# EBonura/bonnie-32

Hardware: AMD Instinct MI355X
Metric: Mtriangles/s + Mpixels/s, 1M-tri synthetic scene @ 2560x1920 (higher is better)
Workload: dtype f32+i32 (exact-order f32 setup/barycentrics, integer snap and RGB555 colour tail); 1 GPU; C3: 1000000 tris @ 2560x1920, 256x256 8-bit atlas, affine+snap+RGB555 dither, painter's; triangles_drawn=485525, fragments=9622635, parallelism=single GPU

## Files before the change

bonnie-32_amd/csrc/b32_api.hip:

```cpp
#include "b32_host.h"
#include "b32_overlay_body.h"

extern "C" {

const char* b32_strerror(int code) {
    switch (code) {
        case B32_OK: return "ok";
        case B32_E_ARG: return "invalid argument";
        case B32_E_INDEX: return "face references a vertex index out of range";
        case B32_E_NAN_KEY: return "NaN painter's-sort key";
        case B32_E_HIP: return "HIP runtime error";
        case B32_E_UNSUPPORTED: return "setting outside the supported hot-path scope";
        case B32_E_NO_DEVICE: return "no HIP device (the rasterizer has no CPU fallback)";
        case B32_E_FRAME_DROPPED: return "an earlier frame in flight ran out of buffer space and drew nothing (deep asynchronous mode)";
        case B32_E_BAND_TIMEOUT: return "a band exchange wait gave up: another rank did not publish / release its frame in time (the frame may hold stale rows)";
        default: return "unknown error";
    }
}

int b32_create(int device, b32_ctx** out) {
    if (!out) return B32_E_ARG;
    *out = nullptr;
    int n = 0;
    if (hipGetDeviceCount(&n) != hipSuccess || n <= 0 || device < 0 || device >= n) return B32_E_NO_DEVICE;
// ... 806 lines not shown
    if ((rc = tmp.alloc(&d_unr, (size_t)K::UNR_ENTRIES))) return rc;
    if ((rc = tmp.alloc(&d_dither, (size_t)16))) return rc;
    launch_constants(c->stream, d_bits, d_unr, d_dither);
    std::vector<uint32_t> h(N);
    HIPCHK(c, hipMemcpyAsync(h.data(), d_bits, N * 4, hipMemcpyDeviceToHost, c->stream));
    if (unr_table257) HIPCHK(c, hipMemcpyAsync(unr_table257, d_unr, K::UNR_ENTRIES, hipMemcpyDeviceToHost, c->stream));
    if (dither16) HIPCHK(c, hipMemcpyAsync(dither16, d_dither, 16 * 4, hipMemcpyDeviceToHost, c->stream));
    HIPCHK(c, hipStreamSynchronize(c->stream));
    for (uint32_t i = 0; i < N && i < cap; ++i) {
        if (names) names[i] = kEntries[i].name;
        if (bits) bits[i] = h[i];
        if (is_f32) is_f32[i] = kEntries[i].f;
    }
    return B32_OK;
}

int b32_last_kernel_times(b32_ctx* c, const char** names, float* ms, uint32_t cap) {
    if (!c || !names || !ms) return 0;
    static const char* const kNames[5] = { "setup", "sort", "bin", "cover", "shade" };
    uint32_t k = 0;
    for (int p = 0; c->phase_frames && p < 5 && k < cap; ++p) {
        if (p != 3 && c->phase_level < 2) continue;
        names[k] = kNames[p]; ms[k] = c->phase_ms[p]; ++k;
    }
    const struct { const char* name; const EventPair* pair; } timers[3] = { { "world_project", &c->world_timer }, { "pick", &c->pick_timer }, { "hover", &c->hover_timer } };
    for (const auto& t : timers) {
        float t_ms = 0.0f;
        if (k < cap && t.pair->elapsed(&t_ms)) { names[k] = t.name; ms[k] = t_ms; ++k; }
    }
    return (int)k;
}

}

extern "C" int b32_set_fragment_counting(b32_ctx* c, int on) {
    if (!c) return B32_E_ARG;
    c->count_fragments = on ? 1 : 0;
    return B32_OK;
}
extern "C" unsigned long long b32_route_count(const b32_ctx* c, int which) {
    if (c && which == 7) return c->pipelined_frames;
    if (c && which == 8) return c->lds_atlas_frames;
    if (c && which == 9) return c->wire_tile_frames;
    if (c && which == 10) return c->span_cover_frames;
    if (c && which == 11) return c->flag_join_frames;
    if (c && which == 12) return c->event_join_frames;
    if (c && which == 13) return c->poll_join_frames;
    if (c && which == 14) return c->lines.tile_batches;
    if (c && which == 15) return c->lines.scan_batches;
    if (c && which == 16) return c->prims.tile_batches;
    if (c && which == 17) return c->prims.scan_batches;
    if (c && which == 18) return c->world_tile_batches;
    if (c && which == 19) return c->world_scan_batches;
    return (c && which >= 0 && which < 8) ? c->routes[which] : 0ull;
}
extern "C" int b32_set_async_depth(b32_ctx* c, int deep) {
    if (!c) return B32_E_ARG;
    if (!deep) { const int rc = settle_pending(c); if (rc) return rc; }
    c->deep_async = deep != 0;
    return B32_OK;
}
extern "C" int b32_set_profiling(b32_ctx* c, int level) {
    if (!c) return B32_E_ARG;
    c->profile_level = level < 0 ? 0 : (level > 2 ? 2 : level);
    if (!c->profile_level) c->hover_timer.timed = c->world_timer.timed = false;
    c->prof_seq = 0;
    if (c->profile_level >= 1 && !c->ev_created) {
        (void)hipSetDevice(c->device);
        for (auto& fr : c->ev) for (auto& e : fr) HIPCHK(c, hipEventCreate(&e));
        c->ev_created = true;
    }
    return B32_OK;
}
extern "C" int b32_set_routes(b32_ctx* c, uint32_t off_mask) {
    if (!c) return B32_E_ARG;
    const int rc = settle_pending(c);
    if (rc) return rc;
    c->route_off = off_mask;
    return B32_OK;
}
extern "C" int b32_set_cheap_threshold(b32_ctx* c, uint32_t den) {
    if (!c || den == 0) return B32_E_ARG;
    c->cheap_den = den;
    c->scene.tex_sig_valid = false;
    return B32_OK;
}
extern "C" int b32_set_pipeline_gate(b32_ctx* c, uint32_t permille) {
    if (!c || permille > 2000u) return B32_E_ARG;
    c->gate_permille = permille;
    return B32_OK;
}
extern "C" int b32_last_shader_clock(const b32_ctx* c, float* ghz, float* fill_ms) {
    if (!c || !ghz) return B32_E_ARG;
    *ghz = 0.0f; if (fill_ms) *fill_ms = 0.0f;
    const unsigned long long* t = c->h_stamps.t;
    if (!t[ST_FILL] || !t[ST_CLKW] || t[ST_CLKW] <= t[ST_FILL] || t[ST_CLK1] <= t[ST_CLK0]) return B32_OK;
    const double ns = (double)(t[ST_CLKW] - t[ST_FILL]) * 10.0;
    *ghz = (float)((double)(t[ST_CLK1] - t[ST_CLK0]) / ns);
    if (fill_ms) *fill_ms = (float)(ns * 1e-6);
    return B32_OK;
}
extern "C" int b32_transparent_counts(const b32_ctx* c, uint32_t* host_bound, uint32_t* device_last) {
    if (!c || !host_bound || !device_last) return B32_E_ARG;
    *host_bound = c->scene.blend_faces; *device_last = c->h_ctrl.n_transparent;
    return B32_OK;
}
// ... 32 lines not shown
```

bonnie-32_amd/csrc/b32_cover.h:

```cpp
#pragma once
#include "b32_fill_common.h"

namespace b32 {

#ifdef B32_TIMELINE
#define B32_DBG_SLOTS(tb) (reinterpret_cast<unsigned long long*>(reinterpret_cast<unsigned char*>(const_cast<uint32_t*>(tb)) + 68096) + (threadIdx.x >> 6) * 32)
#define B32_CLK_DECL(name) unsigned long long name = (unsigned long long)clock64()
#define B32_CLK_ADD(a, slot, from) do { const unsigned long long _n = (unsigned long long)clock64(); if (lane == 0) B32_DBG_SLOTS(tilebuf)[slot] += _n - (from); (from) = _n; } while (0)
#define B32_CNT_ADD(a, slot, v) do { if (lane == 0) B32_DBG_SLOTS(tilebuf)[slot] += (unsigned long long)(v); } while (0)
#else
#define B32_CLK_DECL(name) do { } while (0)
#define B32_CLK_ADD(a, slot, from) do { } while (0)
#define B32_CNT_ADD(a, slot, v) do { } while (0)
#endif

template <int TEXMODE, bool EXACT, bool ZMODE, bool FMT8>
__device__ __forceinline__ uint32_t cover_surface(const Tri& tr, uint32_t cx0, uint32_t cx1, uint32_t cy0, uint32_t cy1, uint32_t li,
                                                  uint32_t* tilebuf, uint32_t x_lo, uint32_t ty_top, uint32_t lane,
                                                  const uint16_t* __restrict__ gtex, const uint16_t* ltex, bool affine) {
    uint32_t drawn_count = 0;
    if (!(tr.flags & F_SLOW)) {
        const uint32_t w = cx1 - cx0, h = cy1 - cy0;
        const uint32_t n88 = ((w + 7) >> 3) * ((h + 7) >> 3), n164 = ((w + 15) >> 4) * ((h + 3) >> 2), n416 = ((w + 3) >> 2) * ((h + 15) >> 4);
        uint32_t sh = 3;
// ... 153 lines not shown
    addr += TRIP; w0 = wa[TRIP - 1] + sa0; w1 = wb[TRIP - 1] + sa1;
}

constexpr float SPAN_MAX_EXT = 512.0f;
constexpr float SPAN_MIN_INV_AREA = 1.0f / 8192.0f;
struct SpanEdge { float r, c; };
__device__ __forceinline__ SpanEdge span_edge(float G) {
    SpanEdge e;
    const float r = __builtin_amdgcn_rcpf(G);
    e.r = G == 0.0f ? -1073741824.0f : r;
    e.c = G == 0.0f ? 64.0f : (G > 0.0f ? -0.5f * r : -0.5f * r + 1.0f);
    return e;
}
__device__ __forceinline__ void span_interval(float E0, float E1, float E2, const SpanEdge& d0, const SpanEdge& d1, const SpanEdge& d2, float wlen,
                                              float& lo, float& hi) {
    const float v0 = __builtin_fmaf(-E0, d0.r, d0.c), v1 = __builtin_fmaf(-E1, d1.r, d1.c), v2 = __builtin_fmaf(-E2, d2.r, d2.c);
    const bool l0 = d0.r > 0.0f, l1 = d1.r > 0.0f, l2 = d2.r > 0.0f;
    lo = fmaxf(fmaxf(l0 ? ceilf(v0) : 0.0f, l1 ? ceilf(v1) : 0.0f), l2 ? ceilf(v2) : 0.0f);
    hi = fminf(fminf(l0 ? wlen : floorf(v0), l1 ? wlen : floorf(v1)), fminf(l2 ? wlen : floorf(v2), wlen));
}
__device__ __forceinline__ void span_trip(unsigned long long* top, unsigned long long* sec, uint32_t addr, uint32_t left, unsigned long long P) {
    constexpr uint32_t TRIP = B32_TRIP;
    if (left) {
        unsigned long long old[TRIP];
#pragma unroll
        for (uint32_t j = 0; j < TRIP; ++j) old[j] = atomicMax(&top[addr + j], j < left ? P : 0ull);
#pragma unroll
        for (uint32_t j = 0; j < TRIP; ++j) atomicMax(&sec[addr + j], j < left ? min(old[j], P) : 0ull);
    }
}

template <int TEXMODE, bool EXACT, int NW, bool ZMODE, bool FMT8, bool P64 = false>
__device__ __forceinline__ unsigned long long phase_a_rows(const FillArgs& a, uint32_t e0, uint32_t n_op, uint32_t lane, uint32_t wave,
                                                           uint32_t* cursor, uint32_t* wmark, const TexDesc& lds_desc,
                                                           uint32_t* tilebuf, const TileRect& rect, const uint16_t* ltex) {
    const uint32_t x_lo = rect.x_lo, x_hi = rect.x_hi, y_lo = rect.y_lo, y_hi = rect.y_hi, ty_top = rect.ty_top;
    const uint16_t* __restrict__ gtex = FMT8 ? reinterpret_cast<const uint16_t*>(a.texels32) : a.texels;
    unsigned long long frags = 0;
    const float ERR = K::ERR;
    const bool affine = a.fp.affine != 0;
    const uint32_t grab_m = max(1u, (n_op + NW * 64u - 1u) / (NW * 64u));
    const uint32_t grab = min(64u, max(4u, (n_op + NW * grab_m - 1u) / (NW * grab_m)));
    for (;;) {
        B32_CLK_DECL(clk);
        uint32_t cs = 0;
        if (lane == 0) cs = atomicAdd(cursor, grab);
        cs = (uint32_t)__builtin_amdgcn_readfirstlane((int)cs);
        if (cs >= n_op) break;
        const uint32_t e = cs + lane;
        bool live = lane < grab && e < n_op;
        Batch b;
        uint32_t my_sid = 0, my_key = 0;
        bool narrow = false;
        load_batch<TEXMODE>(b, a, e0 + e, live, lds_desc, EXACT, ZMODE || (EXACT && !affine), my_sid, my_key, narrow);
        if (ZMODE) { my_key = 0u; my_sid = 0xFFFFFFFEu - my_sid; }
        const uint32_t flags = b.q3.w;
        const uint32_t cx0 = max(b.q1.w & 0xFFFF, x_lo), cx1 = min(b.q1.w >> 16, x_hi);
        const uint32_t cy0 = max(b.q2.x & 0xFFFF, y_lo), cy1 = min(b.q2.x >> 16, y_hi);
        live = live && cx0 < cx1 && cy0 < cy1;
#ifdef B32_TIMELINE
        asm volatile("" :: "v"(cx0), "v"(cy0));
#endif
        B32_CLK_ADD(a, 0, clk); B32_CNT_ADD(a, 4, 1);
        const bool slow = live && (flags & F_SLOW);
        bool span_all = false;
        float sE0 = 0.0f, sE1 = 0.0f;
        uint32_t sG01 = 0, sH01 = 0;
        if (P64 && !EXACT && !ZMODE && a.span_cover) {
            const float fa0 = __uint_as_float(b.q0.z), fb0 = __uint_as_float(b.q0.w), fa1 = __uint_as_float(b.q1.x), fb1 = __uint_as_float(b.q1.y);
            const float inv = __uint_as_float(b.q1.z);
            const float sgn = inv < 0.0f ? -1.0f : 1.0f;
            const float G0 = sgn * fa0, G1 = sgn * fa1, G2 = -(G0 + G1);
            const float H0 = sgn * fb0, H1 = sgn * fb1, H2 = -(H0 + H1);
            const float ext = fmaxf(fmaxf(fmaxf(__builtin_fabsf(G0), __builtin_fabsf(G1)), fmaxf(__builtin_fabsf(H0), __builtin_fabsf(H1))),
                                    fmaxf(__builtin_fabsf(G2), __builtin_fabsf(H2)));
            const float A = __builtin_fabsf(fa0 * fb1 - fb0 * fa1);
            const bool fast = narrow && !(flags & (F_EMPTY | F_SLOW)) && ext <= SPAN_MAX_EXT && __builtin_fabsf(inv) >= SPAN_MIN_INV_AREA && A >= 1.0f;
            span_all = !__ballot(live && !fast);
            const float dx = (float)cx0 - __uint_as_float(b.q0.x), dy = (float)cy0 - __uint_as_float(b.q0.y);
            sE0 = sgn * (fa0 * dx + fb0 * dy); sE1 = sgn * (fa1 * dx + fb1 * dy);
            sG01 = ((uint32_t)hw_cvt_i32(G0) & 0xFFFFu) | ((uint32_t)hw_cvt_i32(G1) << 16);
            sH01 = ((uint32_t)hw_cvt_i32(H0) & 0xFFFFu) | ((uint32_t)hw_cvt_i32(H1) << 16);
        }
        const uint32_t h = (live && !slow) ? cy1 - cy0 : 0u;
        const uint32_t inc = dpp_add_scan(h);
        const uint32_t R = (uint32_t)__builtin_amdgcn_readlane((int)inc, 63);
        const uint32_t P = inc - h;
        const float a0 = __uint_as_float(b.q0.z), b0 = __uint_as_float(b.q0.w), a1 = __uint_as_float(b.q1.x), b1 = __uint_as_float(b.q1.y);
        const uint32_t box = (cx0 - x_lo) | ((cx1 - x_lo) << 8) | ((cy0 - ty_top) << 16);
        const uint32_t boxP = (cx0 - x_lo) | ((cx1 - x_lo) << 6) | ((cy0 - ty_top) << 13) | (P << 19);
        uint32_t lq = 0, lqn = 0;
        auto exact_trip = [&](const Tri& tr, uint32_t& addr, float& w0, float& w1, float sa0, float sa1, float sinv, uint32_t left, unsigned long long P) -> uint32_t {
            unsigned long long* top = reinterpret_cast<unsigned long long*>(tilebuf);
            const uint32_t* mask_l = reinterpret_cast<const uint32_t*>(ltex);
            const bool mask_in_lds = a.mask_lds_words != 0;
            uint32_t drawn = 0;
            float wa[4], wb[4];
            wa[0] = w0; wb[0] = w1;
#pragma unroll
            for (int j = 1; j < 4; ++j) { wa[j] = wa[j - 1] + sa0; wb[j] = wb[j - 1] + sa1; }
            bool in[4]; int ta[4]; unsigned long long Pj[4];
#pragma unroll
            for (int j = 0; j < 4; ++j) {
                const float cx = wa[j] * sinv, cy = wb[j] * sinv;
                const float cz = 1.0f - cx - cy;
                in[j] = ((uint32_t)j < left) & (__builtin_fminf(__builtin_fminf(cx, cy), cz) >= ERR);
                Pj[j] = P; ta[j] = -1;
// ... 330 lines not shown
```

bonnie-32_amd/csrc/b32_device.h:

```cpp
#pragma once
#include <hip/hip_runtime.h>
#include <stdint.h>
#include "../../include/b32raster.h"
#include "b32_world_point.h"

namespace b32 {

constexpr int TILE_W = 64;
constexpr int TILE_H = 64;
constexpr int TILE_STRIDE = 72;
constexpr int FILL_THREADS = 1024;
constexpr int FILL_WAVES = FILL_THREADS / 64;
constexpr uint32_t KEY_INVALID = 0xFFFFFFFFu;

namespace K {
constexpr int      FRAC_BITS = 12;
constexpr float    ONE_F = (float)(1 << FRAC_BITS);
constexpr uint32_t UNR_ENTRIES = 257, UNR_INDEX_OFFSET = 256, UNR_NUMERATOR = 262144, UNR_ROUND_ADD = 1, UNR_ROUND_DIV = 2;
constexpr int32_t  UNR_SUBTRACT = 257;
constexpr uint32_t DIV_D16_SHIFT = 16, DIV_INDEX_SHIFT = 7, DIV_INDEX_MAX = 256, DIV_NR1_SHIFT = 8, DIV_NR2_SHIFT = 8, DIV_SHIFT_BASE = 36;
constexpr uint64_t DIV_INDEX_BIAS = 0x7FC0, DIV_U_ADD = 0x101, DIV_NR1_CONST = 0x2000080, DIV_NR2_CONST = 0x80;
constexpr float    PF_DISTANCE = 5.0f, PF_SCALE = 4.0f, PF_VIEWPORT_DIV = 2.0f, PF_VIEWPORT_FRAC = 0.75f;
constexpr int32_t  PF_DENOM_GUARD = 256;
constexpr float    P_DISTANCE = 5.0f, P_US_SUB = 1.0f, P_VIEWPORT_DIV = 2.0f, P_VIEWPORT_FRAC = 0.75f, P_DENOM_GUARD = 0.001f;
// ... 24 lines not shown
    X("project.distance", F, K::P_DISTANCE) X("project.us_sub", F, K::P_US_SUB) X("project.viewport_div", F, K::P_VIEWPORT_DIV)       \
    X("project.viewport_frac", F, K::P_VIEWPORT_FRAC) X("project.denom_guard", F, K::P_DENOM_GUARD)                                   \
    X("near_plane", F, K::NEAR_PLANE) X("mesh.distance", F, K::MESH_DISTANCE)                                                         \
    X("fill.area_eps", F, K::AREA_EPS) X("fill.err", F, K::ERR) X("fill8.area_eps", F, K::AREA_EPS) X("fill8.err", F, K::ERR)         \
    X("fill.modulate_div", I, K::MOD_DIV) X("fill.modulate_max", I, K::MOD_MAX)                                                       \
    X("fill.shade_clamp_lo", F, K::SHADE_LO) X("fill.shade_clamp_hi", F, K::SHADE_HI) X("fill.shade_max", F, K::SHADE_MAX)            \
    X("fill.nodither_shift", I, K::NODITHER_SHIFT)                                                                                    \
    X("dither.shift", I, K::DITHER_SHIFT) X("dither.clamp_lo", I, K::DITHER_LO) X("dither.clamp_hi", I, K::DITHER_HI)                 \
    X("dither8.shift", I, K::DITHER_SHIFT) X("dither8.clamp_hi", I, K::DITHER_HI) X("dither8.expand_shift", I, K::DITHER8_EXPAND_SHIFT) \
    X("expand5.shl", I, K::EXPAND5_SHL) X("expand5.shr", I, K::EXPAND5_SHR)                                                           \
    X("blend555.in_shift", I, K::BLEND_IN_SHIFT) X("blend555.average_div", I, K::BLEND_AVG_DIV) X("blend555.clamp_hi", I, K::BLEND_HI) \
    X("blend555.clamp_lo", I, K::BLEND_LO) X("blend555.quarter_div", I, K::BLEND_QUARTER_DIV) X("blend555.out_shift", I, K::BLEND_OUT_SHIFT) \
    X("light.min_dist", F, K::LIGHT_MIN_DIST) X("light.color_div", F, K::LIGHT_COLOR_DIV) X("light.total_max", F, K::LIGHT_TOTAL_MAX) \
    X("color15.transparent", I, K::C15_TRANSPARENT) X("color15.black_drawable", I, K::C15_BLACK_DRAWABLE) X("color15.white", I, K::C15_WHITE) \
    X("color15.semi_bit", I, K::C15_SEMI_BIT) X("color15.r_shift", I, K::C15_R_SHIFT) X("color15.g_shift", I, K::C15_G_SHIFT)         \
    X("color15.channel_max", I, K::C15_CHANNEL_MAX)

struct __attribute__((aligned(32))) CovRec {
    uint32_t xy1, xy2, xy3;
    float inv_area;
    uint32_t bbx, bby;
    uint32_t key;
    uint32_t flags;
};
static_assert(sizeof(CovRec) == 32, "CovRec layout");
constexpr uint32_t COV_WIDE = 0x8000u;
struct __attribute__((aligned(64))) ShadeRec {
    float x1, y1, x2, y2;
    float x3, y3, inv_area; uint32_t pk0;
    float u1, u2, u3, v1;
    float v2, v3; uint32_t pk1, pk2;
};
static_assert(sizeof(ShadeRec) == 64, "ShadeRec layout");
constexpr uint32_t SH_BLACK_TR = 1u, SH_DITHER = 2u, SH_SLOW = 4u;
struct __attribute__((aligned(32))) AuxRec {
    float iz1, iz2, iz3, w0_start;
    float w1_start; uint32_t _pad[3];
};
static_assert(sizeof(AuxRec) == 32, "AuxRec layout");

struct RecView { uint4 q0, q1, q2, q3, q4, q5; };
__device__ __forceinline__ float i16lo(uint32_t w) { return (float)(int32_t)(int16_t)(w & 0xFFFFu); }
__device__ __forceinline__ float i16hi(uint32_t w) { return (float)((int32_t)w >> 16); }
__device__ __forceinline__ void view_edges(RecView& r, float x1, float y1, float x2, float y2, float x3, float y3, float inv_area) {
    r.q0 = make_uint4(__float_as_uint(x3), __float_as_uint(y3), __float_as_uint(y2 - y3), __float_as_uint(x3 - x2));
    r.q1.x = __float_as_uint(y3 - y1); r.q1.y = __float_as_uint(x1 - x3); r.q1.z = __float_as_uint(inv_area);
}
__device__ __forceinline__ bool view_from_cov(RecView& r, const uint4& c0, const uint4& c1) {
    r.q1.w = c1.x; r.q2.x = c1.y; r.q3.w = c1.w;
    if ((c0.x & 0xFFFFu) == COV_WIDE) return false;
    view_edges(r, i16lo(c0.x), i16hi(c0.x), i16lo(c0.y), i16hi(c0.y), i16lo(c0.z), i16hi(c0.z), __uint_as_float(c0.w));
    return true;
}
__device__ __forceinline__ void view_edges_from_shade(RecView& r, const uint4& s0, const uint4& s1) {
    view_edges(r, __uint_as_float(s0.x), __uint_as_float(s0.y), __uint_as_float(s0.z), __uint_as_float(s0.w), __uint_as_float(s1.x),
               __uint_as_float(s1.y), __uint_as_float(s1.z));
}
__device__ __forceinline__ uint32_t shade_tex_slot(const uint4& s1, const uint4& s3) { return (s1.w >> 24) | ((s3.z >> 24) << 8); }

constexpr uint32_t F_TEX_MASK   = 0xFFFFu;
constexpr uint32_t F_TEX_NONE   = 0xFFFFu;
constexpr uint32_t F_BLACK_TR   = 1u << 16;
constexpr uint32_t F_BLEND_SHIFT = 17;
constexpr uint32_t F_DITHER     = 1u << 20;
constexpr uint32_t F_SLOW       = 1u << 21;
constexpr uint32_t F_TRANSP     = 1u << 22;
constexpr uint32_t F_EMPTY      = 1u << 23;
constexpr uint32_t F_ALPHA_SHIFT = 24;

struct TexDesc { uint32_t width, height, blend_mode, offset; };

struct Ctrl {
    uint32_t n_visible;
    uint32_t n_transparent;
    uint32_t nan_opaque, nan_transparent;
    uint32_t err_index;
    uint32_t abort;
    uint32_t n_opaque;
    uint32_t n_pairs;
    uint32_t pairs_overflow;
    uint32_t tile_cursor;
    uint32_t list_demand;
    uint32_t need_global_sort;
    uint32_t wire_overflow;
    uint32_t sticky;
    unsigned long long fragments;
};

struct Stamps { unsigned long long t[8]; };
struct Events { uint32_t bad_index, nan_opaque, nan_transparent, overflow, long_transparent, setup_done ,
                join_abort ,
                fill_started ,
                wbin_done ,
                poll_done ,
                poll_lost , _pad[5]; };
__device__ __forceinline__ Events* events_of(Ctrl* ctrl) { return reinterpret_cast<Events*>(reinterpret_cast<unsigned char*>(ctrl) + 128); }
enum { ST_SETUP = 0, ST_BIN = 1, ST_FILL = 2, ST_WIRE = 3, ST_END = 4,
       ST_CLK0 = 5, ST_CLK1 = 6, ST_CLKW = 7 };
__device__ __forceinline__ void phase_stamp(Ctrl* ctrl, int k) {
    if (blockIdx.x == 0 && threadIdx.x == 0) {
        unsigned long long* t = reinterpret_cast<Stamps*>(ctrl + 1)->t;
        if (!t[k]) t[k] = wall_clock64();
    }
}

constexpr uint32_t LOCAL_SORT_CAP = 2048;
// ... 110 lines not shown
    __device__ __forceinline__ bool inside(uint32_t px, uint32_t py) const { return (px < x_hi) & ((py >= y_lo) & (py < y_hi)); }
};
__device__ __forceinline__ TileRect tile_rect(const FrameParams& fp, uint32_t tile) {
    TileRect r;
    r.x_lo = (tile % fp.tiles_x) * TILE_W; r.x_hi = min(r.x_lo + TILE_W, fp.width);
    tile_row_geom(fp, tile / fp.tiles_x, r.ty_top, r.th);
    r.y_lo = max(r.ty_top, fp.band_y0); r.y_hi = min(r.ty_top + r.th, fp.band_y1);
    return r;
}
__device__ __forceinline__ uint32_t pack_tile_span(uint32_t bbx, uint32_t bby, uint32_t flags, const FrameParams& fp, uint32_t& count) {
    count = 0;
    if (flags & F_EMPTY) return 0xFFFFFFFFu;
    const uint32_t min_x = bbx & 0xFFFF, max_x = bbx >> 16;
    const uint32_t min_y = max(bby & 0xFFFF, fp.band_y0), max_y = min(bby >> 16, fp.band_y1);
    if (min_x >= max_x || min_y >= max_y) return 0xFFFFFFFFu;
    const uint32_t tx0 = min_x / TILE_W, tx1 = (max_x - 1) / TILE_W;
    const uint32_t ty0 = tile_row_of(fp, min_y), ty1 = tile_row_of(fp, max_y - 1);
    count = (tx1 - tx0 + 1) * (ty1 - ty0 + 1);
    return tx0 | (tx1 << 8) | (ty0 << 16) | (ty1 << 24);
}

struct SortScratch {
    uint32_t* block_hist;
    uint32_t  max_blocks;
    uint32_t* digit_total;
};
constexpr int SORT_THREADS = 256;
constexpr int SORT_ITEMS = 16;
constexpr int SORT_TILE = SORT_THREADS * SORT_ITEMS;

struct RadixExtra {
    Ctrl* post_ctrl = nullptr; const uint32_t* partials = nullptr; uint32_t npart = 0;
    uint32_t* ranges_out = nullptr; uint32_t n_ranges = 0;
};
void launch_radix_pass(hipStream_t s, const uint32_t* keys_in, const uint32_t* vals_in, uint32_t* keys_out, uint32_t* vals_out,
                       const uint32_t* n_dev, uint32_t n_cap, int shift, int bits, const SortScratch& sc, const RadixExtra& ex = RadixExtra());

constexpr uint32_t LIGHTS_INLINE = 8;
struct LightSet { B32Light l[LIGHTS_INLINE]; };
constexpr uint32_t BATCH_MESHES = 32;
struct MeshRow { float ambient; uint32_t flags; B32Fog fog; };
struct MeshTable { MeshRow m[BATCH_MESHES]; };
constexpr uint32_t ROW_CULL = 1u, ROW_FOG = 2u, ROW_PLACED = 4u;
struct PlaceTable { B32Placement p[BATCH_MESHES]; };
static_assert(sizeof(B32Placement) == 20 && sizeof(PlaceTable) == 640, "B32Placement layout");
struct RecArrays { CovRec* cov; ShadeRec* shade; AuxRec* aux; };
#ifndef B32_FILL_PAD
#define B32_FILL_PAD 32
#endif
constexpr uint32_t FILL_PAD = B32_FILL_PAD;
struct DirectBin {
    uint32_t* fill;
    uint32_t* lists;
    uint32_t region, cap_opaque, cap_transparent;
    uint32_t with_class;
    uint32_t epoch;
};
void launch_merge_mesh(hipStream_t s, const B32Vertex* sv, uint32_t nv, const B32Face* sf, uint32_t nf, uint32_t nt, B32Vertex* dv, B32Face* df,
                       uint32_t vbase, uint32_t tbase, uint32_t mesh);
void launch_offset_tex(hipStream_t s, const TexDesc* src, uint32_t nt, TexDesc* dst, uint32_t texel_base);
struct SetupBuffers {
    const B32Vertex* verts;
    const B32Face* faces;
    const TexDesc* tex;
    const B32Light* lights;
    RecArrays recs;
    DirectBin db;
    float* shades;
    uint32_t* keys;
    uint32_t* spans;
    uint32_t* partials;
    Ctrl* ctrl;
    WireTri* wire;
    const float* pos12;
    const float* attr12;
    uint32_t* face_of;
};
struct SetupArgs {
    FrameParams fp;
    SetupBuffers buf;
    LightSet lset;
    MeshTable mtab;
    PlaceTable ptab;
};
void launch_setup(hipStream_t s, const SetupArgs& a);
void launch_gate(hipStream_t s, Ctrl* prev, uint32_t need, uint32_t patience_ticks, uint32_t start_seq, Ctrl* mine, uint32_t start_patience_ticks = 200000000u);
void launch_flag(hipStream_t s, Ctrl* ctrl, uint32_t epoch);
void launch_flag_poll(hipStream_t s, Ctrl* ctrl, uint32_t seq);
void launch_flag_wbin(hipStream_t s, Ctrl* ctrl, uint32_t epoch);
void launch_join(hipStream_t s, Ctrl* ctrl, uint32_t epoch, uint32_t patience_ticks);
void launch_pack_streams(hipStream_t s, const B32Vertex* verts, uint32_t nv, float* pos12, float* attr12, bool with_lit);
void launch_pose_rest(hipStream_t s, const B32Vertex* verts, uint32_t nv, float* rest);
void launch_pose(hipStream_t s, const float* rest, const uint16_t* bone_of, B32Vertex* verts, uint32_t nv, const B32Bone* bones, uint32_t n_bones);
void launch_project_fixed(hipStream_t s, const float* pos, uint32_t n, B32Camera cam, uint32_t w, uint32_t h,
                          int32_t* sx, int32_t* sy, float* z);
void launch_selftest(hipStream_t s, int op, const float* a, const float* b, const float* c, float* out, uint32_t n);
void launch_constants(hipStream_t s, uint32_t* consts, uint8_t* unr, int32_t* dither);
void launch_build_mask(hipStream_t s, const uint16_t* texels15, const uint32_t* texels32, uint32_t n, uint32_t* mask);
constexpr uint32_t MASK_LDS_MAX_WORDS = 9216;
void launch_clear(hipStream_t s, uint32_t* fb, size_t n_px, uint32_t rgba);
struct UploadSegs { void* dst[16]; uint32_t src_off[16]; uint32_t n16[16]; uint32_t count; };
void launch_upload(hipStream_t s, const void* arena_dev, const UploadSegs& segs);
void launch_ctrl_out(hipStream_t s, Ctrl* ctrl, void* dst128);
void launch_expand_indexed(hipStream_t s, const uint8_t* idx, uint32_t n, const uint16_t* clut, uint32_t clut_len, uint16_t* out, uint32_t* skippable);

void launch_bin(hipStream_t s, const FrameParams& fp, const uint32_t* spans, const uint32_t* order, Ctrl* ctrl,
// ... 63 lines not shown
    const float* pos; uint32_t stride, nv;
    const HoverHalfEdge* he; const uint32_t* poly_start; const uint32_t* poly_verts; uint32_t np, nh;
    OverlayPoint* tab;
    OverlayBounds* bounds;
    const uint32_t* selected; uint32_t n_sel;
    B32MeshOverlay o;
    uint32_t at_brackets, at_edges, at_dots, at_hover_vertex, at_hover_edge, at_hover_face, at_selected, at_preview;
    uint32_t hover_face_cnt;
    uint32_t g_edges, g_pedges, g_sel, g_pfaces, g_hover, g_brackets;
};
void launch_overlay(hipStream_t s, const OverlayArgs& a);
constexpr uint32_t BLEND_SORT_CAP = 2048;
bool bin_spans_applicable(const FrameParams& fp, const SortScratch& sc, bool with_class);
bool launch_bin_spans(hipStream_t s, const FrameParams& fp, const uint32_t* spans, const uint32_t* keys, const uint32_t* partials, Ctrl* ctrl,
                      const SortScratch& sc, uint32_t pair_cap, uint32_t* ranges, uint32_t* tile_mid, uint32_t blend_cap, uint32_t* pair_vals);
void launch_tile_ranges(hipStream_t s, const uint32_t* pair_keys, const Ctrl* ctrl, uint32_t pair_cap, uint32_t* ranges, uint32_t n_keys);

void launch_clear_gradient(hipStream_t s, uint32_t* fb, float* zbuf, uint32_t width, uint32_t height, uint32_t y0, uint32_t y1, uint32_t top, uint32_t bottom);
void launch_sky(hipStream_t s, const B32SkyVertex* v, uint32_t nv, const uint32_t* faces, uint32_t nf, const B32Camera& cam, float2* proj,
                uint32_t* fb, uint32_t width, uint32_t height, uint32_t band_y0, uint32_t band_y1);
void launch_stars(hipStream_t s, const int32_t* cx, const int32_t* cy, const uint8_t* rgb, uint32_t n, float size, uint32_t* fb,
                  uint32_t width, uint32_t height, uint32_t band_y0, uint32_t band_y1);
void launch_upscale_nearest(hipStream_t s, const uint32_t* src, uint32_t sw, uint32_t sh, uint32_t* dst, uint32_t dw, uint32_t dh);

struct FillArgs {
    FrameParams fp;
    const CovRec* crecs;
    const ShadeRec* srecs;
    const AuxRec* xrecs;
    const float* shades;
    uint32_t* pair_vals;
    const uint32_t* keys;
    uint32_t local_sort;
    const uint32_t* ranges;
    uint32_t* tile_mid;
    uint32_t tile_keys_only;
    const TexDesc* tex;
    const uint16_t* texels;
    uint32_t* fb;
    float* zbuf;
    uint32_t* vis;
    TexDesc tex0;
    Ctrl* ctrl;
    uint32_t lds_tex_texels;
    uint32_t may_blend;
    uint32_t exact_coverage;
    uint32_t skip_solid;
    const uint32_t* texels32;
    uint32_t ordered_all;
    uint32_t gather_blend;
    uint32_t inline_bin;
    uint32_t direct_bin;
    uint32_t* tile_fill;
    uint32_t epoch;
    uint32_t list_stride;
    const uint32_t* spans;
    const uint32_t* partials;
    const uint32_t* texmask;
    uint32_t mask_lds_words;
    uint32_t clear_on, clear_rgba;
    uint32_t clear_depth;
    uint32_t wide;
    const uint8_t* atlas0;
    uint32_t atlas_idx_bytes;
    uint32_t stagger;
    uint32_t span_cover;
    uint32_t join_seq, join_patience;
    uint32_t start_seq;
    uint32_t start_defer;
    uint32_t fused;
#ifdef B32_TIMELINE
    unsigned long long* dbg;
#endif
};
void launch_fill(hipStream_t s, const FillArgs& a, int n_cu, hipEvent_t after_cover = nullptr);
size_t fill_lds_tex_budget();
constexpr uint32_t ATLAS_CLUT_BYTES = 512;
uint32_t fill_lds_atlas_room(bool wide);

}
```

bonnie-32_amd/csrc/b32_fill.hip:

```cpp
#include "b32_cover.h"
#include "b32_shade_tile.h"

namespace b32 {

constexpr uint32_t RQ_WORDS = 64, RQ_BYTES = RQ_WORDS * 4;
static_assert(2 * (4 * LDS_TILE_BYTES + LDS_MISC_BYTES + 8 * RQ_BYTES + 511) / 512 * 512 <= 160 * 1024, "two 8-wave workgroups per CU");

template <int NT>
__device__ __forceinline__ void reduce_setup_counters(const FillArgs& a, uint32_t* misc, uint32_t tid, uint32_t lane) {
    if (tid < 5) misc[8 + tid] = 0;
    __syncthreads();
    const uint32_t npart = (a.fp.nf + 255) / 256;
    uint32_t acc[5] = { 0, 0, 0, 0, 0 };
    for (uint32_t b = tid; b < npart; b += NT)
#pragma unroll
        for (int k = 0; k < 5; ++k) acc[k] += a.partials[b * 8 + k];
#pragma unroll
    for (int k = 0; k < 5; ++k) {
        const uint32_t tot = (uint32_t)__builtin_amdgcn_readlane((int)dpp_add_scan(acc[k]), 63);
        if (lane == 0 && tot) atomicAdd(&misc[8 + k], tot);
    }
    __syncthreads();
    if (tid == 0) {
        const uint32_t t[5] = { misc[8], misc[9], misc[10], misc[11], misc[12] };
// ... 37 lines not shown
        const unsigned long long t0 = wall_clock64();
        uint32_t lost = 0, waited = 0;
        while (__hip_atomic_fetch_add(&ev->poll_done, 0u, __ATOMIC_RELAXED, __HIP_MEMORY_SCOPE_AGENT) != a.join_seq) {
            if (wall_clock64() - t0 > (unsigned long long)a.join_patience) { lost = 1; break; }
            waited = 1;
            __builtin_amdgcn_s_sleep(32);
        }
        if (lost) { atomicOr(&a.ctrl->sticky, 8u); (void)__hip_atomic_exchange(&ev->poll_lost, a.join_seq, __ATOMIC_RELAXED, __HIP_MEMORY_SCOPE_AGENT); }
        if (waited) __builtin_amdgcn_fence(__ATOMIC_ACQUIRE, "agent");
        misc[7] = lost;
    }
    __syncthreads();
    return misc[7] != 0;
}

template <int NT>
__device__ __forceinline__ TexDesc stage_texture(const FillArgs& a, unsigned char* dst_bytes, uint32_t tid) {
    const TexDesc lds_desc = a.tex[0];
    const uint4* src = reinterpret_cast<const uint4*>(a.texels + lds_desc.offset);
    uint4* dst = reinterpret_cast<uint4*>(dst_bytes);
    const uint32_t nq = (a.lds_tex_texels + 7) / 8;
    for (uint32_t i = tid; i < nq; i += NT) dst[i] = src[i];
    return lds_desc;
}

template <int NT>
__device__ __forceinline__ void leave_undrawn(const FillArgs& a, uint32_t ntiles, uint32_t tid, uint32_t redraw, bool publish) {
    if (a.direct_bin) {
        for (uint32_t t = blockIdx.x * NT + tid; t < ntiles; t += gridDim.x * NT) {
            uint32_t* fl = a.tile_fill + (size_t)t * FILL_PAD;
            if (redraw & 2u) atomicMax(&a.ctrl->list_demand, fl[0]);
            fl[0] = 0; fl[1] = 0;
        }
        if (blockIdx.x == 0 && tid == 0 && publish) a.ctrl->need_global_sort = redraw;
    }
    if (a.clear_on) clear_band<NT>(a);
}

__device__ __forceinline__ void staggered_start(const FillArgs& a) {
    if (blockIdx.x >= gridDim.x / 2) {
        const unsigned long long t0 = wall_clock64();
        while (wall_clock64() - t0 < (unsigned long long)a.stagger) __builtin_amdgcn_s_sleep(8);
    }
}

template <int TEXMODE, int NT, bool P64>
__device__ __forceinline__ bool tile_list_range(const FillArgs& a, uint32_t tile, uint32_t* tilebuf, uint32_t* sort_cnt, uint32_t* misc, uint32_t tid,
                                                uint32_t& e0, uint32_t& e1) {
    if (P64 && a.inline_bin) {
        e0 = e1 = tile * a.list_stride;
    } else if (P64 && a.direct_bin) {
        const uint32_t* fl = a.tile_fill + (size_t)tile * FILL_PAD;
        const uint32_t n_o = fl[0], n_t = fl[1];
        e0 = tile * a.list_stride; e1 = e0 + n_o;
        if (tid == 0) {
            if (a.gather_blend) a.tile_mid[tile] = e0 + a.list_stride - n_t;
            if (n_o | n_t) atomicAdd(&a.ctrl->n_pairs, n_o + n_t);
        }
    } else if (P64) {
        e0 = a.ranges[tile]; e1 = a.gather_blend ? a.tile_mid[tile] : a.ranges[tile + 1];
    } else if (TEXMODE == 0 && a.local_sort) {
        e0 = a.ranges[tile];
        const uint32_t e2 = a.ranges[tile + 1];
        if (e2 - e0 > LOCAL_SORT_CAP) {
            if (tid == 0) atomicOr(&a.ctrl->need_global_sort, 1u);
            __syncthreads();
            return false;
        }
        if (e2 > e0) [[clang::noinline]] tile_local_sort<NT>(tilebuf, sort_cnt, misc + 8, a.keys, a.pair_vals + e0, e2 - e0, &misc[4]);
        e1 = e0 + misc[4];
        if (tid == 0) a.tile_mid[tile] = e1;
    } else {
        e0 = a.ranges[2 * tile]; e1 = a.ranges[2 * tile + 1];
    }
    return true;
}

template <int NT>
__device__ __forceinline__ void collect_tile_list(const FillArgs& a, uint32_t tile, uint32_t e0, uint32_t* misc, uint32_t pre_span, uint32_t pre_key,
                                                  uint32_t tid, uint32_t lane) {
    const FrameParams& fp = a.fp;
    const uint32_t txi = tile % fp.tiles_x, tyl = tile / fp.tiles_x;
    const uint32_t r_end = e0 + a.list_stride;
    for (uint32_t f0 = 0; f0 < fp.nf; f0 += NT) {
        const uint32_t f = f0 + tid;
        bool hit = false, tr = false;
        if (f < fp.nf) {
            const uint32_t span = f0 == 0 ? pre_span : a.spans[f];
            hit = span != 0xFFFFFFFFu && txi >= (span & 0xFF) && txi <= ((span >> 8) & 0xFF) && tyl >= ((span >> 16) & 0xFF) && tyl <= (span >> 24);
            if (hit && a.gather_blend) tr = ((f0 == 0 ? pre_key : a.keys[f]) >> 31) != 0;
        }
        const unsigned long long mo = __ballot(hit && !tr), mt = __ballot(hit && tr);
        uint32_t bo = 0, bt = 0;
        if (lane == 0 && mo) bo = atomicAdd((&misc[4]), (uint32_t)__builtin_popcountll(mo));
        if (lane == 0 && mt) bt = atomicAdd((&misc[5]), (uint32_t)__builtin_popcountll(mt));
        bo = (uint32_t)__builtin_amdgcn_readfirstlane((int)bo); bt = (uint32_t)__builtin_amdgcn_readfirstlane((int)bt);
        const unsigned long long below = (1ull << lane) - 1ull;
        if (hit && !tr) a.pair_vals[e0 + bo + (uint32_t)__builtin_popcountll(mo & below)] = f;
        if (hit && tr) a.pair_vals[r_end - 1u - (bt + (uint32_t)__builtin_popcountll(mt & below))] = f;
    }
}

template <bool EXACT, int NT, bool ZMODE, bool P64>
__device__ __forceinline__ void seed_planes(const FillArgs& a, uint32_t* tilebuf, const TileRect& rect, uint32_t tid) {
    const FrameParams& fp = a.fp;
    if (P64 && ZMODE) {
        unsigned long long* t64 = reinterpret_cast<unsigned long long*>(tilebuf);
        for (uint32_t p = tid; p < TILE_W * rect.th; p += NT) {
            const uint32_t row = p >> 6, col = p & 63;
// ... 362 lines not shown
```

bonnie-32_amd/csrc/b32_fill_common.h:

```cpp
#pragma once
#include "b32_device.h"
#ifndef B32_TRIP
#define B32_TRIP 4
#endif
#ifndef B32_DRAIN_TRIPS
#define B32_DRAIN_TRIPS 2
#endif
static_assert(B32_DRAIN_TRIPS > 0, "row remainders are queued and worked off at most B32_DRAIN_TRIPS trips per round");
#ifndef B32_P64_WAVES
#define B32_P64_WAVES 4
#endif
#ifndef B32_P64_STRIDE
#define B32_P64_STRIDE 66
#endif

namespace b32 {

constexpr int LDS_TILE_BYTES = TILE_H * TILE_STRIDE * 4;
constexpr int STR64 = B32_P64_STRIDE;
static_assert(STR64 >= 64 && STR64 <= TILE_STRIDE && (TILE_H - 1) * STR64 + 64 + 4 <= TILE_H * TILE_STRIDE, "64-bit planes must fit their allocation, trip overshoot included");
constexpr int LDS_MISC_BYTES = 64;
constexpr int LDS_MARK_BYTES = FILL_WAVES * 64 * 4;
constexpr int LDS_TEX_OFFSET = 2 * LDS_TILE_BYTES + LDS_MISC_BYTES + LDS_MARK_BYTES;
constexpr int LDS_SORT_CNT_BYTES = 8 * 256 * 4;
// ... 187 lines not shown
            case B32_BLEND_ADD_QUARTER: r = min(b + f / 4, 255); break;
            case B32_BLEND_ERASE:       r = 0; a8 = 0; break;
        }
        ps1 |= (uint32_t)r << (8 * i);
    }
    if (alpha < 255) {
        const float a = (float)alpha / 255.0f, inv_a = 1.0f - a;
        uint32_t o = 0xFF000000u;
#pragma unroll
        for (int i = 0; i < 3; ++i)
            o |= f2u8_sat((float)((ps1 >> (8 * i)) & 255) * a + (float)((back >> (8 * i)) & 255) * inv_a) << (8 * i);
        return o;
    }
    return ps1 | (a8 << 24);
}

__device__ __forceinline__ void replay_w(const Tri& t, uint32_t px, uint32_t py, float& w0, float& w1) {
    float r0 = t.w0_start, r1 = t.w1_start;
    for (uint32_t y = t.min_y; y < py; ++y) { r0 += t.b0; r1 += t.b1; }
    for (uint32_t x = t.min_x; x < px; ++x) { r0 += t.a0; r1 += t.a1; }
    w0 = r0; w1 = r1;
}
__device__ __forceinline__ void edge_w(const Tri& t, uint32_t px, uint32_t py, float& w0, float& w1) {
    if (!(t.flags & F_SLOW)) {
        const float dx = (float)px - t.x3, dy = (float)py - t.y3;
        w0 = t.a0 * dx + t.b0 * dy; w1 = t.a1 * dx + t.b1 * dy;
    } else replay_w(t, px, py, w0, w1);
}

struct Batch {
    uint4 q0, q1, q2, q3, q4, q5;
    uint32_t tw, th, toff;
};

__device__ __forceinline__ void load_shade_view(const FillArgs& a, uint32_t sid, bool need5, RecView& r) {
    const uint4* sp = reinterpret_cast<const uint4*>(a.srecs + sid);
    const uint4 s0 = sp[0], s1 = sp[1], s2 = sp[2], s3 = sp[3];
    view_edges_from_shade(r, s0, s1);
    r.q1.w = 0; r.q2.x = 0;
    r.q2.y = s2.x; r.q2.z = s2.y; r.q2.w = s2.z;
    r.q3.x = s2.w; r.q3.y = s3.x; r.q3.z = s3.y;
    const uint32_t sh = s3.w >> 24;
    r.q3.w = shade_tex_slot(s1, s3) | ((sh & SH_BLACK_TR) ? F_BLACK_TR : 0u) | ((sh & SH_DITHER) ? F_DITHER : 0u) | ((sh & SH_SLOW) ? F_SLOW : 0u) |
             (255u << F_ALPHA_SHIFT);
    r.q4 = make_uint4(s1.w & 0xFFFFFFu, s3.z & 0xFFFFFFu, s3.w & 0xFFFFFFu, 0u);
    r.q5 = make_uint4(0, 0, 0, 0);
    if (need5 || (sh & SH_SLOW)) {
        const uint4* xp = reinterpret_cast<const uint4*>(a.xrecs + sid);
        const uint4 x0 = xp[0], x1 = xp[1];
        r.q4.w = x0.w; r.q5 = make_uint4(x1.x, x0.x, x0.y, x0.z);
    }
    if (sh & SH_SLOW) { const uint4 c1 = reinterpret_cast<const uint4*>(a.crecs + sid)[1]; r.q1.w = c1.x; r.q2.x = c1.y; }
}
__device__ __forceinline__ void load_full_view(const FillArgs& a, uint32_t sid, RecView& r) {
    load_shade_view(a, sid, true, r);
    const uint4 c1 = reinterpret_cast<const uint4*>(a.crecs + sid)[1];
    r.q1.w = c1.x; r.q2.x = c1.y; r.q3.w = c1.w;
}

template <int TEXMODE>
__device__ __forceinline__ void load_batch(Batch& b, const FillArgs& a, uint32_t entry, bool live, const TexDesc& lds_desc, bool need_uv,
                                           bool need_aux, uint32_t& sid_out, uint32_t& key_out, bool& narrow_out) {
    b.q0 = b.q1 = b.q2 = b.q3 = b.q4 = b.q5 = make_uint4(0, 0, 0, 0);
    b.tw = b.th = b.toff = 0;
    sid_out = 0; key_out = 0; narrow_out = false;
    if (live) {
        const uint32_t sid = a.pair_vals[entry];
        const uint4* cp = reinterpret_cast<const uint4*>(a.crecs + sid);
        const uint4 c0 = cp[0], c1 = cp[1];
        sid_out = sid; key_out = c1.z;
        RecView v;
        v.q0 = v.q1 = v.q2 = v.q3 = v.q4 = v.q5 = make_uint4(0, 0, 0, 0);
        const bool narrow = view_from_cov(v, c0, c1);
        narrow_out = narrow;
        if (!narrow || need_uv) {
            const uint4* sp = reinterpret_cast<const uint4*>(a.srecs + sid);
            const uint4 s0 = sp[0], s1 = sp[1];
            if (!narrow) view_edges_from_shade(v, s0, s1);
            if (need_uv) {
                const uint4 s2 = sp[2], s3 = sp[3];
                v.q2.y = s2.x; v.q2.z = s2.y; v.q2.w = s2.z;
                v.q3.x = s2.w; v.q3.y = s3.x; v.q3.z = s3.y;
                v.q4 = make_uint4(s1.w & 0xFFFFFFu, s3.z & 0xFFFFFFu, s3.w & 0xFFFFFFu, 0u);
                const uint32_t tid = c1.w & F_TEX_MASK;
                if (tid != F_TEX_NONE) {
                    if (TEXMODE == 1) { b.tw = lds_desc.width; b.th = lds_desc.height; b.toff = 0; }
                    else { const TexDesc d = a.tex[tid]; b.tw = d.width; b.th = d.height; b.toff = d.offset; }
                }
            }
        }
        if (need_aux || (c1.w & F_SLOW)) {
            const uint4* xp = reinterpret_cast<const uint4*>(a.xrecs + sid);
            const uint4 x0 = xp[0], x1 = xp[1];
            v.q4.w = x0.w; v.q5 = make_uint4(x1.x, x0.x, x0.y, x0.z);
        }
        b.q0 = v.q0; b.q1 = v.q1; b.q2 = v.q2; b.q3 = v.q3; b.q4 = v.q4; b.q5 = v.q5;
    }
}
__device__ __forceinline__ Tri tri_from_batch(const Batch& b, int t, bool full) {
    Tri r;
    r.x3 = bcf(__uint_as_float(b.q0.x), t); r.y3 = bcf(__uint_as_float(b.q0.y), t);
    r.a0 = bcf(__uint_as_float(b.q0.z), t); r.b0 = bcf(__uint_as_float(b.q0.w), t);
    r.a1 = bcf(__uint_as_float(b.q1.x), t); r.b1 = bcf(__uint_as_float(b.q1.y), t);
    r.inv_area = bcf(__uint_as_float(b.q1.z), t);
    const uint32_t bbx = bcu(b.q1.w, t), bby = bcu(b.q2.x, t);
    r.min_x = bbx & 0xFFFF; r.max_x = bbx >> 16; r.min_y = bby & 0xFFFF; r.max_y = bby >> 16;
    r.flags = bcu(b.q3.w, t);
    r.u1 = r.u2 = r.u3 = r.v1 = r.v2 = r.v3 = 0.0f; r.tw = r.th = r.toff = 0; r.w0_start = r.w1_start = 0.0f;
    if (full) {
        r.u1 = bcf(__uint_as_float(b.q2.y), t); r.u2 = bcf(__uint_as_float(b.q2.z), t); r.u3 = bcf(__uint_as_float(b.q2.w), t);
        r.v1 = bcf(__uint_as_float(b.q3.x), t); r.v2 = bcf(__uint_as_float(b.q3.y), t); r.v3 = bcf(__uint_as_float(b.q3.z), t);
        r.tw = bcu(b.tw, t); r.th = bcu(b.th, t); r.toff = bcu(b.toff, t);
    }
    if (r.flags & F_SLOW) { r.w0_start = bcf(__uint_as_float(b.q4.w), t); r.w1_start = bcf(__uint_as_float(b.q5.x), t); }
    r.iz1 = r.iz2 = r.iz3 = 0.0f;
    if (full) { r.iz1 = bcf(__uint_as_float(b.q5.y), t); r.iz2 = bcf(__uint_as_float(b.q5.z), t); r.iz3 = bcf(__uint_as_float(b.q5.w), t); }
    return r;
}
__device__ __forceinline__ Tri tri_from_view(const RecView& r, bool with_uv) {
    Tri t;
    t.x3 = __uint_as_float(r.q0.x); t.y3 = __uint_as_float(r.q0.y); t.a0 = __uint_as_float(r.q0.z); t.b0 = __uint_as_float(r.q0.w);
    t.a1 = __uint_as_float(r.q1.x); t.b1 = __uint_as_float(r.q1.y); t.inv_area = __uint_as_float(r.q1.z);
    t.min_x = r.q1.w & 0xFFFF; t.max_x = r.q1.w >> 16; t.min_y = r.q2.x & 0xFFFF; t.max_y = r.q2.x >> 16;
    t.flags = r.q3.w;
    t.w0_start = __uint_as_float(r.q4.w); t.w1_start = __uint_as_float(r.q5.x);
    t.u1 = t.u2 = t.u3 = t.v1 = t.v2 = t.v3 = 0.0f; t.iz1 = t.iz2 = t.iz3 = 0.0f; t.tw = t.th = t.toff = 0;
    if (with_uv) {
        t.u1 = __uint_as_float(r.q2.y); t.u2 = __uint_as_float(r.q2.z); t.u3 = __uint_as_float(r.q2.w);
        t.v1 = __uint_as_float(r.q3.x); t.v2 = __uint_as_float(r.q3.y); t.v3 = __uint_as_float(r.q3.z);
        t.iz1 = __uint_as_float(r.q5.y); t.iz2 = __uint_as_float(r.q5.z); t.iz3 = __uint_as_float(r.q5.w);
    }
    return t;
}
template <bool EXACT, bool ZMODE>
__device__ __forceinline__ void commit_fragment(uint32_t* tilebuf, uint32_t addr, uint32_t li, uint32_t zkey) {
    if (ZMODE) atomicMin(reinterpret_cast<unsigned long long*>(tilebuf) + addr, ((unsigned long long)zkey << 32) | li);
    else if (EXACT) atomicMax(&tilebuf[addr], li);
    else {
        const uint32_t old = atomicMax(&tilebuf[addr], li);
        atomicMax(&tilebuf[addr + TILE_H * TILE_STRIDE], min(old, li));
    }
}
__device__ __forceinline__ bool frag_zkey(const Tri& t, float bcx, float bcy, float bcz, uint32_t& zkey) {
    const float inv_z = bcx * t.iz1 + bcy * t.iz2 + bcz * t.iz3;
    const float z = rcp_exact(inv_z);
    zkey = zsort_key(z);
    return z == z;
}

__device__ inline float exact_depth_at(const FillArgs& a, uint32_t sid, uint32_t px, uint32_t py) {
    RecView rv;
    load_full_view(a, sid, rv);
    const Tri tr = tri_from_view(rv, true);
    float w0, w1, bcx, bcy, bcz;
    edge_w(tr, px, py, w0, w1);
    (void)inside_bc(tr, w0, w1, bcx, bcy, bcz);
    const float inv_z = bcx * tr.iz1 + bcy * tr.iz2 + bcz * tr.iz3;
    return rcp_exact(inv_z);
}

struct Hit { float bcx, bcy, bcz; uint32_t texel, vc1, vc2, vc3, flags, sid; };
template <bool FMT8>
__device__ __forceinline__ bool hit_test(const FillArgs& a, uint32_t sid, uint32_t px, uint32_t py, Hit& h) {
    RecView rv;
    load_shade_view(a, sid, a.fp.affine == 0, rv);
    Tri tr = tri_from_view(rv, true);
    const uint32_t txid = tr.flags & F_TEX_MASK;
    if (txid != F_TEX_NONE) {
        if (a.fp.nt == 1) { tr.tw = a.tex0.width; tr.th = a.tex0.height; tr.toff = a.tex0.offset; }
        else { const TexDesc d = a.tex[txid]; tr.tw = d.width; tr.th = d.height; tr.toff = d.offset; }
    }
    float w0, w1;
    edge_w(tr, px, py, w0, w1);
    if (!inside_bc(tr, w0, w1, h.bcx, h.bcy, h.bcz)) return false;
    h.texel = 0;
    if (!texel_drawn<0, FMT8>(tr, h.bcx, h.bcy, h.bcz, FMT8 ? reinterpret_cast<const uint16_t*>(a.texels32) : a.texels, nullptr, h.texel, a.fp.affine != 0)) return false;
    h.vc1 = rv.q4.x; h.vc2 = rv.q4.y; h.vc3 = rv.q4.z; h.flags = tr.flags; h.sid = sid;
    return true;
}
template <bool FMT8>
__device__ __forceinline__ uint32_t colour(const FillArgs& a, const Hit& h, int shading, uint32_t px, uint32_t py) {
    float shv[9];
    if (shading != B32_SHADE_NONE) for (int j = 0; j < 9; ++j) shv[j] = a.shades[(size_t)h.sid * 9 + j];
    if (FMT8) return (shade8(h.texel, h.bcx, h.bcy, h.bcz, h.vc1, h.vc2, h.vc3, h.flags, shading, shv, px, py) & 0xFFFFFFu) | 0xFF000000u;
    return shade15<true>(h.texel, h.bcx, h.bcy, h.bcz, h.vc1, h.vc2, h.vc3, h.flags, shading, shv, px, py);
}

using RecRegs = RecView;
__device__ __forceinline__ void rec_load(const FillArgs& a, uint32_t sid, bool need5, RecRegs& r) { load_shade_view(a, sid, need5, r); }
__device__ __forceinline__ bool hit_prepare(const FillArgs& a, const RecRegs& r, uint32_t px, uint32_t py, Hit& h, int& taddr) {
    Tri tr = tri_from_view(r, true);
    float w0, w1;
    edge_w(tr, px, py, w0, w1);
    taddr = -1;
    if (!inside_bc(tr, w0, w1, h.bcx, h.bcy, h.bcz)) return false;
    h.vc1 = r.q4.x; h.vc2 = r.q4.y; h.vc3 = r.q4.z; h.flags = tr.flags;
    const uint32_t txid = tr.flags & F_TEX_MASK;
    if (txid == F_TEX_NONE) return true;
    TexDesc d;
    if (a.fp.nt == 1) d = a.tex0; else d = a.tex[txid];
    if (d.width == 0 || d.height == 0) { taddr = -2; return true; }
    float u, v;
    interp_uv(h.bcx, h.bcy, h.bcz, tr.u1, tr.u2, tr.u3, tr.v1, tr.v2, tr.v3, tr.iz1, tr.iz2, tr.iz3, a.fp.affine != 0, u, v);
    taddr = (int)(d.offset + texel_index(u, v, d.width, d.height));
    return true;
// ... 63 lines not shown
```

bonnie-32_amd/csrc/b32_frame.hip:

```cpp
#include "b32_host.h"

static void swap_with(b32_ctx* c, FrameSet& a) { std::swap(c->cur, a); }
static void rotate_sets(b32_ctx* c) {
    swap_with(c, c->alt[0]);
    if (c->n_sets == 3) std::swap(c->alt[0], c->alt[1]);
}
static void unrotate_sets(b32_ctx* c) {
    if (c->n_sets == 3) std::swap(c->alt[0], c->alt[1]);
    swap_with(c, c->alt[0]);
}
static int pipeline_ensure(b32_ctx* c) {
    if (!c->side) {
        int prio_least = 0, prio_greatest = 0;
        (void)hipDeviceGetStreamPriorityRange(&prio_least, &prio_greatest);
        HIPCHK(c, hipStreamCreateWithPriority(&c->side, hipStreamNonBlocking, prio_least));
        HIPCHK(c, hipEventCreateWithFlags(&c->ev_main, hipEventDisableTiming));
        HIPCHK(c, hipEventCreateWithFlags(&c->ev_wbin, hipEventDisableTiming));
        HIPCHK(c, hipEventCreateWithFlags(&c->cur.ev_setup, hipEventDisableTiming));
        for (FrameSet& a : c->alt) HIPCHK(c, hipEventCreateWithFlags(&a.ev_setup, hipEventDisableTiming));
        c->side_dirty = true;
    }
    for (uint32_t k = 0; k + 1 < c->n_sets; ++k) {
        FrameSet& a = c->alt[k];
        if (!a.d_ctrl) {
            HIPCHK(c, hipMalloc(reinterpret_cast<void**>(&a.d_ctrl), sizeof(Ctrl) + sizeof(Stamps) + sizeof(Events)));
            HIPCHK(c, hipMemsetAsync(a.d_ctrl, 0, sizeof(Ctrl) + sizeof(Stamps) + sizeof(Events), c->stream));
            c->side_dirty = true;
        }
        if (a.cap_work < c->cap_work || !a.crecs) {
            HIPCHK(c, hipStreamSynchronize(c->stream));
            a.release();
            const size_t n = c->cap_work;
            int rc;
            if ((rc = ensure_plain(c, a.keys0, n))) return rc;
            if ((rc = ensure_plain(c, a.crecs, n))) return rc;
            if ((rc = ensure_plain(c, a.srecs, n))) return rc;
            if ((rc = ensure_plain(c, a.xrecs, n))) return rc;
            if ((rc = ensure_plain(c, a.spans, n))) return rc;
            if ((rc = ensure_plain(c, a.face_of, n))) return rc;
            if ((rc = ensure_plain(c, a.partials, (size_t)((n + 255) / 256) * 8 + 8))) return rc;
            a.cap_work = n;
        }
    }
    return B32_OK;
}

extern "C" {
int validate_settings(const B32Settings* st) {
    if (st->shading > B32_SHADE_GOURAUD) return B32_E_ARG;
    if (st->n_lights && !st->lights) return B32_E_ARG;
    if (st->shading != B32_SHADE_NONE)
        for (uint32_t i = 0; i < st->n_lights; ++i)
            if (st->lights[i].enabled && st->lights[i].type > B32_LIGHT_SPOT) return B32_E_ARG;
    return B32_OK;
}

static uint32_t bits_for(uint32_t n_keys) { uint32_t b = 1; while ((1ull << b) < n_keys) ++b; return b; }

struct FramePlan {
    bool wire_back = false, wire_front = false;
    bool with_class = false;
    bool ordered_all = false;
    bool want_prio64 = false;
    bool exact_cov = false;
    bool local_sort = false;
    bool want_inline = false;
    bool direct_bin = false;
    bool inline_bin = false, prio64 = false;
    uint32_t list_stride = 0;
    DirectBin db{};
    uint32_t ntiles = 0;
    bool fused = false, wide = false;
    void set_prio64(bool on) { prio64 = on; fused = plan_fused(prio64, wire_front, ordered_all); }
    HandOver hand_over_kind = HandOver::None;
    hipStream_t setup_stream = nullptr;
    uint32_t poll_seq = 0, poll_patience = 0;
    uint32_t start_seq = 0;
    bool wire_on = false, wire_binned = false, wire_polled = false;
    WireArgs wa{};
    const float *pos12 = nullptr, *attr12 = nullptr;
    bool prof_all = false, prof_fill = false;
    hipEvent_t* ev = nullptr;
    int pair_buf = 0;
};

struct SetsGuard {
    b32_ctx* c; bool armed = false;
    explicit SetsGuard(b32_ctx* ctx) : c(ctx) {}
    SetsGuard(const SetsGuard&) = delete;
    SetsGuard& operator=(const SetsGuard&) = delete;
    void rotate() { rotate_sets(c); armed = true; }
    void dismiss() { armed = false; }
    ~SetsGuard() { if (armed) { unrotate_sets(c); c->pipelined = false; } }
};

static FrameParams frame_params(const b32_ctx* c, const B32Camera* cam, const B32Settings* st, const B32Fog* fog, bool wire_any) {
    FrameParams fp{};
    fp.cam = *cam;
    fp.width = c->width; fp.height = c->height;
    fp.band_y0 = c->band_y0; fp.band_y1 = c->band_y1;
    fp.tiles_x = (c->width + TILE_W - 1) / TILE_W;
    fp.tile_h = TILE_H;
    fp.tile_yb = (c->band_y0 / TILE_H) * TILE_H;
    fp.tiles_y = c->band_y1 > c->band_y0 ? (c->band_y1 - fp.tile_yb + TILE_H - 1) / TILE_H : 0;
    fp.nv = c->scene.nv; fp.nf = c->scene.nf; fp.nt = c->scene.nt;
    fp.n_lights = st->shading != B32_SHADE_NONE ? st->n_lights : 0;
    fp.ambient = st->ambient;
    fp.affine = st->affine_textures; fp.shading = st->shading; fp.backface_cull = st->backface_cull;
    fp.dithering = st->dithering; fp.fixed_point = st->use_fixed_point; fp.has_fog = fog ? 1 : 0; fp.zmode = st->use_zbuffer ? 1 : 0;
    if (fog) fp.fog = *fog;
    fp.camfx = make_camfx_any(*cam, c->width, c->height);
    fp.fmt8 = c->scene.fmt8 ? 1 : 0;
    fp.ortho = st->has_ortho ? 1 : 0; fp.xray = st->xray_mode ? 1 : 0;
    fp.ortho_zoom = st->ortho_zoom; fp.ortho_cx = st->ortho_center_x; fp.ortho_cy = st->ortho_center_y;
    fp.wire_collect = wire_any ? 1 : 0;
    fp.band_only = 0;
    fp.redraw = c->redrawing ? 1 : 0;
    fp.tex_blend_any = c->scene.tex_blend_any ? 1 : 0;
    fp.batched = c->frame_batched ? 1 : 0;
    fp.placed = c->frame_placed ? 1 : 0;
// ... 74 lines not shown
            if (wt > c->cur.cap_wire_tiles || !c->cur.wire_fill) {
                if ((rc = ensure_plain(c, c->cur.wire_fill, (wt + 2) * FILL_PAD + 64))) return rc;
                if ((rc = ensure_plain(c, c->cur.wire_lists, wt * WIRE_TILE_CAP + 64))) return rc;
                c->cur.cap_wire_tiles = wt; c->cur.wire_grid = 0;
            }
            const unsigned long long grid = ((unsigned long long)c->width << 40) ^ ((unsigned long long)c->band_y0 << 20) ^ c->band_y1;
            if (grid != c->cur.wire_grid) {
                HIPCHK(c, hipMemsetAsync(c->cur.wire_fill, 0, ((c->cur.cap_wire_tiles + 2) * FILL_PAD + 64) * sizeof(uint32_t), s));
                c->cur.wire_grid = grid; c->side_dirty = true;
            }
        }
    }
    return B32_OK;
}

static int plan_route(b32_ctx* c, FrameParams& fp, const SortScratch& sc, FramePlan& r) {
    const bool wire_front = r.wire_front;
    int rc;
    r.with_class = c->scene.may_blend && !c->scene.fmt8;
    const bool spans_ok = !(c->route_off & B32_ROUTE_SORT_FREE) && c->scene.local_sort_ok && bin_spans_applicable(fp, sc, r.with_class);
    r.ordered_all = c->scene.fmt8 ? c->scene.blend8 : (fp.xray != 0);
    r.want_prio64 = spans_ok && !fp.ortho && !r.ordered_all;
    if (r.want_prio64 && !(c->route_off & B32_ROUTE_CUT_TILES)) {
        static_assert(PLAN_TILE_H == (uint32_t)TILE_H, "b32_frame_plan.h cuts the tiles of b32_device.h");
        const TileGrid g = plan_cut_grid(fp.tiles_x, c->band_y0, c->band_y1, (uint32_t)c->n_cu, (uint32_t)B32_MIN_TILE_H);
        fp.tile_h = g.tile_h; fp.tile_yb = g.tile_yb; fp.tiles_y = g.tiles_y;
    }
    const uint32_t ntiles = r.ntiles = fp.tiles_x * fp.tiles_y;
    r.exact_cov = c->count_fragments || !c->scene.cheap_ok || (fp.zmode && !r.want_prio64);
    r.local_sort = !r.exact_cov && c->scene.local_sort_ok && !fp.ortho && !r.ordered_all && !fp.zmode;
    fp.band_only = (r.want_prio64 && c->band_set) ? 1 : 0;
    r.list_stride = (c->scene.nf + 31u) & ~31u;
    r.want_inline = r.want_prio64 && !wire_front && c->scene.nf <= (r.with_class ? 2048u : 8192u) && (size_t)ntiles * r.list_stride <= ((size_t)4 << 20) &&
                    !(c->route_off & B32_ROUTE_INLINE_BIN);
    if (c->scene.direct_ntiles != ntiles) { c->scene.direct_ntiles = ntiles; c->scene.direct_cap_opaque = 0; c->scene.direct_ok = true; }
    if (r.want_prio64 && !r.want_inline && !wire_front && c->scene.direct_ok && !(c->route_off & B32_ROUTE_DIRECT_BIN) && ntiles) {
        if (!c->scene.direct_cap_opaque) c->scene.direct_cap_opaque = std::max<uint32_t>(512u, (uint32_t)std::min<uint64_t>((uint64_t)3 * c->scene.nf / ntiles + 64, 1u << 24));
        if (c->scene.nf <= 65536u && (uint64_t)ntiles * (c->scene.nf + (r.with_class ? BLEND_SORT_CAP : 0u)) <= (8u << 20)) c->scene.direct_cap_opaque = std::max(c->scene.direct_cap_opaque, c->scene.nf);
        const uint32_t cap_o = (c->scene.direct_cap_opaque + 31u) & ~31u;
        const uint32_t region = cap_o + (r.with_class ? BLEND_SORT_CAP : 0u);
        const size_t need = (size_t)ntiles * region + 64;
        if (need <= ((size_t)1 << 28)) {
            if (need > c->cur.cap_direct || !c->cur.direct_lists) {
                if ((rc = ensure_plain(c, c->cur.direct_lists, need + need / 8))) return rc;
                c->cur.cap_direct = need + need / 8;
            }
            const size_t need_fill = (size_t)ntiles * FILL_PAD + 64;
            if (need_fill > c->cur.cap_tile_fill || !c->cur.tile_fill) {
                if ((rc = ensure_plain(c, c->cur.tile_fill, need_fill * 2))) return rc;
                c->cur.cap_tile_fill = need_fill * 2;
                HIPCHK(c, hipMemsetAsync(c->cur.tile_fill, 0, c->cur.cap_tile_fill * sizeof(uint32_t), c->stream));
                c->side_dirty = true;
            }
            if (++c->epoch == 0) c->epoch = 1;
            r.db.fill = c->cur.tile_fill; r.db.lists = c->cur.direct_lists; r.db.region = region; r.db.cap_opaque = cap_o;
            r.db.cap_transparent = r.with_class ? BLEND_SORT_CAP : 0u; r.db.with_class = r.with_class ? 1u : 0u; r.db.epoch = c->epoch;
            r.direct_bin = true;
            r.list_stride = region;
        } else c->scene.direct_ok = false;
    }
    if (!r.direct_bin && r.want_inline) {
        const size_t need = (size_t)ntiles * r.list_stride + 64;
        if (need > c->cap_inline) {
            if ((rc = ensure_plain(c, c->inline_lists, need + need / 2))) return rc;
            c->cap_inline = need + need / 2;
        }
        r.inline_bin = true;
    }
    r.set_prio64(r.direct_bin || r.inline_bin);
    return B32_OK;
}

static int frame_positions(b32_ctx* c, const FrameParams& fp, const float*& pos12, const float*& attr12) {
    int rc;
    pos12 = attr12 = nullptr;
    if (c->scene.nv && c->scene.nf > 8192u && !(c->route_off & B32_ROUTE_PACKED_STREAMS)) {
        const bool want_lit = fp.shading != B32_SHADE_NONE;
        if ((!c->scene.pos_valid || (want_lit && !c->scene.lit_valid)) && c->scene.band_frames >= 1) {
            const bool with_lit = want_lit || c->scene.lit_valid;
            const size_t need = (size_t)c->scene.nv * (with_lit ? 12 : 6);
            if (need > c->scene.cap_pos12 || !c->scene.d_pos12) {
                if ((rc = ensure_plain(c, c->scene.d_pos12, need + 16))) return rc;
                c->scene.cap_pos12 = need;
            }
            launch_pack_streams(c->stream, c->scene.d_verts, c->scene.nv, c->scene.d_pos12, c->scene.d_pos12 + (size_t)c->scene.nv * 3, with_lit);
            c->scene.pos_valid = true; c->scene.lit_valid = with_lit; c->side_dirty = true;
        }
        c->scene.band_frames++;
        if (c->scene.pos_valid && (!want_lit || c->scene.lit_valid)) { pos12 = c->scene.d_pos12; attr12 = c->scene.d_pos12 + (size_t)c->scene.nv * 3; }
    }
    return B32_OK;
}

static int bin_keyed(b32_ctx* c, const FrameParams& fp, FramePlan& r, const SortScratch& sc, hipEvent_t ev_bin) {
    hipStream_t s = c->stream;
    const uint32_t ntiles = r.ntiles;
    int& cur = r.pair_buf;
    cur = 0;
    if (r.local_sort) {
        if (ev_bin) HIPCHK(c, hipEventRecord(ev_bin, s));
        launch_bin_faces(s, fp, c->cur.spans, c->cur.keys0, c->cur.partials, c->cur.d_ctrl, c->pkeys[0], c->pvals[0], (uint32_t)c->cap_pairs, 0);
    } else {
        RadixExtra ex1; ex1.post_ctrl = c->cur.d_ctrl; ex1.partials = c->cur.partials; ex1.npart = (c->scene.nf + 255) / 256;
        launch_radix_pass(s, c->cur.keys0, nullptr, c->keys1, c->vals[1], c->scene.d_consts, c->scene.nf, 0, 8, sc, ex1);
        launch_radix_pass(s, c->keys1, c->vals[1], c->cur.keys0, c->vals[0], &c->cur.d_ctrl->n_visible, c->scene.nf, 8, 8, sc);
        launch_radix_pass(s, c->cur.keys0, c->vals[0], c->keys1, c->vals[1], &c->cur.d_ctrl->n_visible, c->scene.nf, 16, 8, sc);
        launch_radix_pass(s, c->keys1, c->vals[1], c->cur.keys0, c->vals[0], &c->cur.d_ctrl->n_visible, c->scene.nf, 24, 8, sc);
        if (fp.ortho) {
            launch_class_keys(s, c->cur.crecs, c->vals[0], &c->cur.d_ctrl->n_visible, c->scene.nf, c->cur.keys0);
            launch_radix_pass(s, c->cur.keys0, c->vals[0], c->keys1, c->vals[1], &c->cur.d_ctrl->n_visible, c->scene.nf, 0, 8, sc);
            HIPCHK(c, hipMemcpyAsync(c->vals[0], c->vals[1], (size_t)c->scene.nf * 4, hipMemcpyDeviceToDevice, s));
        }
        if (ev_bin) HIPCHK(c, hipEventRecord(ev_bin, s));
        launch_bin(s, fp, c->cur.spans, c->vals[0], c->cur.d_ctrl, c->counts, c->block_sums, c->bin_blocks, c->pkeys[0], c->pvals[0], (uint32_t)c->cap_pairs);
    }
    const uint32_t n_sort_keys = r.local_sort ? ntiles : 2 * ntiles;
    const uint32_t kb = bits_for(n_sort_keys ? n_sort_keys : 1);
    if (kb <= 8 || kb > 12) {
        for (uint32_t shift = 0; shift < kb; shift += 8) {
            launch_radix_pass(s, c->pkeys[cur], c->pvals[cur], c->pkeys[cur ^ 1], c->pvals[cur ^ 1], &c->cur.d_ctrl->n_pairs, (uint32_t)c->cap_pairs, (int)shift, 8, sc);
            cur ^= 1;
        }
        launch_tile_ranges(s, c->pkeys[cur], c->cur.d_ctrl, (uint32_t)c->cap_pairs, c->ranges, n_sort_keys);
    } else {
        RadixExtra exr; exr.ranges_out = c->ranges; exr.n_ranges = n_sort_keys + 1;
        launch_radix_pass(s, c->pkeys[cur], c->pvals[cur], c->pkeys[cur ^ 1], c->pvals[cur ^ 1], &c->cur.d_ctrl->n_pairs, (uint32_t)c->cap_pairs, 0, kb <= 11 ? 11 : 12, sc, exr);
        cur ^= 1;
    }
    return B32_OK;
}

static FillArgs fill_args(const b32_ctx* c, const FrameParams& fp, const FramePlan& r) {
    FillArgs fa{};
    fa.fp = fp; fa.crecs = c->cur.crecs; fa.srecs = c->cur.srecs; fa.xrecs = c->cur.xrecs; fa.shades = c->cur.shades; fa.pair_vals = c->pvals[r.pair_buf]; fa.ranges = c->ranges;
    fa.keys = c->cur.keys0; fa.local_sort = r.local_sort ? 1u : 0u; fa.tile_keys_only = (r.local_sort || r.prio64) ? 1u : 0u; fa.tile_mid = c->tile_mid;
    fa.tex = c->scene.d_tex; fa.texels = c->scene.d_texels; fa.fb = c->fb; fa.vis = c->vis; fa.zbuf = c->zbuf; fa.ctrl = c->cur.d_ctrl;
    fa.tex0 = c->scene.nt ? c->scene.h_tex[0] : TexDesc{ 0, 0, 0, 0 };
    fa.lds_tex_texels = 0;
    if (c->scene.nt == 1 && r.exact_cov) {
        const size_t n = (size_t)c->scene.h_tex[0].width * c->scene.h_tex[0].height;
        if (n > 0 && n * 2 <= fill_lds_tex_budget()) fa.lds_tex_texels = (uint32_t)n;
    }
    fa.exact_coverage = r.exact_cov ? 1u : 0u;
    fa.may_blend = c->scene.may_blend ? 1u : 0u;
    fa.skip_solid = r.wire_front ? 1u : 0u;
    fa.texels32 = c->scene.d_texels32;
    fa.ordered_all = r.ordered_all ? 1u : 0u;
    fa.fused = r.fused ? 1u : 0u;
    fa.wide = r.wide ? 1u : 0u;
    fa.texmask = c->scene.d_texmask;
    { const uint32_t words = c->scene.pool_texels / 32 + 2; fa.mask_lds_words = (c->scene.pool_texels && words <= MASK_LDS_MAX_WORDS) ? words : 0u; }
    fa.inline_bin = r.inline_bin ? 1u : 0u; fa.list_stride = r.list_stride; fa.spans = c->cur.spans; fa.partials = c->cur.partials;
    if (r.inline_bin) fa.pair_vals = c->inline_lists;
    fa.direct_bin = r.direct_bin ? 1u : 0u; fa.tile_fill = c->cur.tile_fill; fa.epoch = c->epoch;
    if (r.direct_bin) fa.pair_vals = c->cur.direct_lists;
    fa.gather_blend = (r.prio64 && r.with_class) ? 1u : 0u;
    fa.stagger = (c->route_off & B32_ROUTE_STAGGER) ? 0u : 1u;
    fa.span_cover = (r.prio64 && !r.exact_cov && !fp.zmode && !(c->route_off & B32_ROUTE_SPAN_COVER)) ? 1u : 0u;
    fa.atlas0 = c->scene.d_atlas0; fa.atlas_idx_bytes = 0;
    if (r.prio64 && !c->scene.fmt8 && c->scene.nt == 1 && c->scene.atlas_idx_bytes && !(c->route_off & B32_ROUTE_LDS_ATLAS) &&
        c->scene.atlas_idx_bytes + ATLAS_CLUT_BYTES + 16u <= fill_lds_atlas_room(r.wide))
        fa.atlas_idx_bytes = c->scene.atlas_idx_bytes;
    if (c->scene.fmt8) fa.fp.xray = 0;
    return fa;
}

static int choose_frame_set(b32_ctx* c, const FramePlan& r, SetsGuard& sets) {
    c->pipelined = false;
    const uint32_t pipe_min_faces = 2048u;
    if (!(c->frame_pending && c->pipe_hint && !c->redrawing && !r.prof_all && c->scene.nf > pipe_min_faces && !(c->route_off & B32_ROUTE_PIPELINE) &&
          c->stream != hipStreamLegacy))
        return B32_OK;
    int rc;
    if ((rc = pipeline_ensure(c))) return rc;
    sets.rotate();
    c->pipelined = true;
    if (c->join_stream != c->stream) {
        int pm = 0, ps = 0;
        c->join_ok = hipStreamGetPriority(c->stream, &pm) == hipSuccess && hipStreamGetPriority(c->side, &ps) == hipSuccess && pm != ps;
        c->join_stream = c->stream;
    }
    return B32_OK;
}

static int profiling_row(b32_ctx* c, FramePlan& r) {
    if (!r.prof_fill) return B32_OK;
    if (!c->ev_created) {
        for (auto& fr : c->ev) for (auto& e : fr) if (hipEventCreate(&e) != hipSuccess) return B32_E_HIP;
        c->ev_created = true;
    }
    r.ev = c->ev[c->ev_frames % EV_RING];
    return B32_OK;
}

static void plan_pipeline(b32_ctx* c, const FrameParams& fp, FramePlan& r) {
    const bool join_small = !c->frame_batched && (c->join_stream != c->stream || c->join_ok);
    c->pipe_hint = plan_pipe_hint(r.direct_bin, r.ntiles, (uint32_t)c->n_cu, c->frame_batched, join_small);
    if (!c->pipe_hint) c->pipelined = false;
    c->last_local_sort = r.local_sort || r.want_prio64;
    c->last_exact = r.ordered_all ? true : (r.exact_cov && !fp.zmode);
    c->last_direct = r.direct_bin;
    const bool narrow_only = (c->route_off & B32_ROUTE_WIDE_GROUPS) != 0;
    r.wide = plan_wide(r.ntiles, (uint32_t)c->n_cu, narrow_only);
    r.hand_over_kind = plan_hand_over({ c->pipelined, c->frame_batched, c->join_ok, r.direct_bin, r.wire_front, r.ordered_all, r.ntiles, (uint32_t)c->n_cu, narrow_only });
}

static int reset_ctrl_of_empty_frame(b32_ctx* c) {
    if (c->scene.nf) return B32_OK;
// ... 47 lines not shown
    b.recs = RecArrays{ c->cur.crecs, c->cur.srecs, c->cur.xrecs }; b.db = r.db;
    b.shades = c->cur.shades; b.keys = c->cur.keys0;
    b.spans = r.direct_bin ? nullptr : c->cur.spans;
    b.partials = c->cur.partials; b.ctrl = c->cur.d_ctrl; b.wire = c->cur.wire;
    b.pos12 = r.pos12; b.attr12 = r.attr12; b.face_of = c->cur.face_of;
    return a;
}

static bool take_lost_flag(b32_ctx* c) {
    const bool lose_flag = (c->inject & 1u) != 0;
    c->inject &= ~1u;
    return lose_flag;
}

static int hand_over(b32_ctx* c, FramePlan& r) {
    hipStream_t s = c->stream;
    if (r.hand_over_kind == HandOver::Poll) {
        const bool lose_flag = take_lost_flag(c);
        if (++c->join_seq == 0) c->join_seq = 1;
        launch_flag_poll(c->side, c->cur.d_ctrl, lose_flag ? c->join_seq ^ 0x40000000u : c->join_seq);
        r.poll_seq = c->join_seq; r.poll_patience = lose_flag ? PATIENCE_INJECTED_TICKS : PATIENCE_TICKS;
        c->flag_join_frames++; c->poll_join_frames++;
    } else if (r.hand_over_kind == HandOver::FlagJoin) {
        const bool lose_flag = take_lost_flag(c);
        launch_flag(c->side, c->cur.d_ctrl, lose_flag ? c->epoch ^ 0x40000000u : c->epoch);
        launch_join(s, c->cur.d_ctrl, c->epoch, lose_flag ? PATIENCE_INJECTED_TICKS : PATIENCE_TICKS);
        c->flag_join_frames++;
    } else if (r.hand_over_kind == HandOver::Event) {
        hipError_t e1 = hipEventRecord(c->cur.ev_setup, c->side);
        if (e1 == hipSuccess) e1 = hipStreamWaitEvent(s, c->cur.ev_setup, 0);
        if (e1 != hipSuccess) { (void)hipStreamSynchronize(c->side); c->last_hip = (int)e1; return B32_E_HIP; }
        c->event_join_frames++;
    }
    if (c->pipelined && r.wire_on && r.wa.tile_fill) {
        launch_wire_bin(c->side, r.wa, r.wire_back, r.wire_front, true);
        if (r.wire_back) { launch_flag_wbin(c->side, c->cur.d_ctrl, r.wa.epoch); r.wire_polled = true; }
        else HIPCHK(c, hipEventRecord(c->ev_wbin, c->side));
        r.wire_binned = true;
    }
    c->cur.in_flight = true;
    if (r.prof_all) HIPCHK(c, hipEventRecord(r.ev[1], s));
    return B32_OK;
}

static int tile_lists(b32_ctx* c, const FrameParams& fp, const SortScratch& sc, FramePlan& r) {
    hipStream_t s = c->stream;
    int rc;
    if (r.prof_all && r.want_prio64) HIPCHK(c, hipEventRecord(r.ev[2], s));
    if (r.want_prio64 && !r.prio64)
        r.set_prio64(launch_bin_spans(s, fp, c->cur.spans, r.with_class ? c->cur.keys0 : nullptr, c->cur.partials, c->cur.d_ctrl, sc, (uint32_t)c->cap_pairs, c->ranges,
                                      c->tile_mid, BLEND_SORT_CAP, c->pvals[0]));
    if (!r.prio64 && (rc = bin_keyed(c, fp, r, sc, r.prof_all ? r.ev[2] : nullptr))) return rc;
    c->routes[r.direct_bin ? 0 : r.inline_bin ? 1 : r.prio64 ? 2 : 3]++;
    const bool direct_safe = r.direct_bin && r.db.cap_opaque >= c->scene.nf && (!r.with_class || c->scene.blend_faces <= BLEND_SORT_CAP);
    c->pending_may_redraw = !(r.inline_bin || direct_safe);
    if (r.prof_fill) HIPCHK(c, hipEventRecord(r.ev[3], s));
    return B32_OK;
}

static int fill(b32_ctx* c, const FrameParams& fp, FramePlan& r) {
    const bool fused = r.fused;
    int rc;
    FillArgs fa = fill_args(c, fp, r);
    if (++c->fill_seq == 0) c->fill_seq = 1;
    fa.start_seq = r.start_seq = c->fill_seq;
    fa.join_seq = r.poll_seq; fa.join_patience = r.poll_patience;
    if ((c->inject & 2u) && fused && r.ntiles) { c->inject &= ~2u; fa.start_seq = 0; c->start_lost = true; }
    fa.start_defer = (fused && r.ntiles > 2u * (uint32_t)c->n_cu && fa.gather_blend) ? 1u : 0u;
    if (c->clear_pending) {
        const bool has_z = c->zbuf && c->zbuf_valid;
        if (fused && (!has_z || fp.zmode) && c->scene.nf && r.ntiles && c->clear_y0 == c->band_y0 && c->clear_y1 == c->band_y1) {
            fa.clear_on = 1; fa.clear_rgba = c->clear_rgba; fa.clear_depth = (has_z && fp.zmode) ? 1u : 0u; c->clear_pending = false;
        } else if ((rc = flush_clear(c))) return rc;
    }
    if (fa.atlas_idx_bytes && fused) c->lds_atlas_frames++;
    if (fa.span_cover && fused) c->span_cover_frames++;
    launch_fill(c->stream, fa, c->n_cu, r.prof_fill ? r.ev[4] : nullptr);
    return B32_OK;
}

static int wire_phases(b32_ctx* c, FramePlan& r) {
    hipStream_t s = c->stream;
    if (r.wire_on && r.wire_binned && !r.wire_polled) HIPCHK(c, hipStreamWaitEvent(s, c->ev_wbin, 0));
    if (r.wire_on) launch_wire(s, r.wa, r.wire_back, r.wire_front, r.wire_binned, r.wire_polled ? c->cur.d_ctrl : nullptr, r.wa.epoch);
    if (r.prof_all) HIPCHK(c, hipEventRecord(r.ev[5], s));
    if (r.prof_fill) c->ev_frames++;
    return B32_OK;
}

static void remember_cover(b32_ctx* c, const FramePlan& r) {
    const uint32_t tiles = r.fused ? r.ntiles : 0u;
    b32_ctx::CoverOf* slot = &c->cover_of[0];
    for (auto& co : c->cover_of) { if (co.ctrl == c->cur.d_ctrl) { slot = &co; break; } if (!co.ctrl) slot = &co; }
    *slot = { c->cur.d_ctrl, tiles, std::min<uint32_t>(r.ntiles, (uint32_t)c->n_cu * 2u), tiles ? r.start_seq : 0u };
}

int enqueue_frame(b32_ctx* c, const B32Camera* cam, const B32Settings* st, const B32Fog* fog) {
    FramePlan r;
    r.wire_back = st->backface_cull && st->backface_wireframe;
    r.wire_front = st->wireframe_overlay != 0;
    FrameParams fp = frame_params(c, cam, st, fog, r.wire_back || r.wire_front);
    LightSet lset{};
    r.prof_fill = c->profile_level >= 1 && (c->prof_seq++ % c->prof_stride) == 0;
    r.prof_all = r.prof_fill && c->profile_level >= 2;
    int rc;
    SetsGuard sets(c);
// ... 197 lines not shown
```

bonnie-32_amd/csrc/b32_frame_plan.h:

```cpp
#pragma once
#include <cstdint>

namespace b32 {

constexpr uint32_t PATIENCE_TICKS = 200000000u;
constexpr uint32_t PATIENCE_INJECTED_TICKS = 200000u;

constexpr uint32_t PLAN_TILE_H = 64;
struct TileGrid { uint32_t tile_h, tile_yb, tiles_y; };
inline TileGrid plan_cut_grid(uint32_t tiles_x, uint32_t band_y0, uint32_t band_y1, uint32_t n_cu, uint32_t min_tile_h) {
    uint32_t th = PLAN_TILE_H;
    if (band_y1 <= band_y0) return { th, (band_y0 / th) * th, 0u };
    while (th > min_tile_h && tiles_x * ((band_y1 + th - 1) / th - band_y0 / th) < (th == PLAN_TILE_H ? 2u : 1u) * n_cu &&
           (band_y1 - band_y0) / (th / 2) + 2 <= 255 ) th /= 2;
    const uint32_t yb = (band_y0 / th) * th;
    return { th, yb, (band_y1 - yb + th - 1) / th };
}

inline uint32_t plan_gate_need(uint32_t gate_permille, uint32_t tiles, uint32_t groups) {
    if (!gate_permille || !tiles) return 0u;
    const uint32_t pre = tiles > groups ? tiles - groups : 0u;
    return gate_permille > 1000u ? (uint32_t)((uint64_t)(gate_permille - 1000u) * pre / 1000u)
                                 : pre + (uint32_t)((uint64_t)(gate_permille - 1u) * groups / 1000u);
}

inline bool plan_fused(bool prio64, bool wire_front, bool ordered_all) { return prio64 && !wire_front && !ordered_all; }

inline bool plan_wide(uint32_t ntiles, uint32_t n_cu, bool narrow_only) { return ntiles <= n_cu && !narrow_only; }

inline bool plan_pipe_hint(bool direct_bin, uint32_t ntiles, uint32_t n_cu, bool batched, bool join_small) {
    return direct_bin && (ntiles > 2u * n_cu || batched || join_small);
}

enum class HandOver {
    None,
    Poll,
    FlagJoin,
    Event
};
struct HandOverIn {
    bool pipelined;
    bool batched;
    bool join_ok;
    bool direct_bin, wire_front, ordered_all;
    uint32_t ntiles, n_cu;
    bool narrow_only;
};
inline HandOver plan_hand_over(const HandOverIn& in) {
    if (!in.pipelined) return HandOver::None;
    if (in.batched && in.join_ok && plan_fused(in.direct_bin, in.wire_front, in.ordered_all) && in.ntiles && 8u * in.ntiles <= 5u * in.n_cu &&
        !in.narrow_only)
        return HandOver::Poll;
    if (in.direct_bin && in.join_ok && !in.batched) return HandOver::FlagJoin;
    return HandOver::Event;
}

}
```

bonnie-32_amd/csrc/b32_host.h:

```cpp
#pragma once
#include "b32_device.h"
#include "b32_frame_plan.h"
#include <algorithm>
#include <cstdio>
#include <chrono>
#include <cstring>
#include <vector>

using namespace b32;
#ifndef B32_MIN_TILE_H
#define B32_MIN_TILE_H 8
#endif

namespace {
constexpr int EV_RING = 64;
constexpr int EV_PER_FRAME = 6;
}

struct FrameSet {
    uint32_t* keys0 = nullptr; CovRec* crecs = nullptr; ShadeRec* srecs = nullptr; AuxRec* xrecs = nullptr;
    uint32_t* spans = nullptr; uint32_t* partials = nullptr; size_t cap_work = 0;
    uint32_t* face_of = nullptr;
    float* shades = nullptr; size_t cap_shades = 0;
    uint32_t* direct_lists = nullptr; size_t cap_direct = 0;
    uint32_t* tile_fill = nullptr; size_t cap_tile_fill = 0;
    WireTri* wire = nullptr; size_t cap_wire = 0;
    uint32_t *wire_fill = nullptr, *wire_lists = nullptr; size_t cap_wire_tiles = 0;
    unsigned long long wire_grid = 0;
    Ctrl* d_ctrl = nullptr;
    hipEvent_t ev_setup = nullptr;
    bool in_flight = false;
    void release() {
        for (void* p : { (void*)keys0, (void*)crecs, (void*)srecs, (void*)xrecs, (void*)spans, (void*)face_of, (void*)partials, (void*)shades,
                         (void*)direct_lists, (void*)tile_fill, (void*)wire, (void*)wire_fill, (void*)wire_lists }) if (p) (void)hipFree(p);
        FrameSet e; e.d_ctrl = d_ctrl; e.ev_setup = ev_setup; e.in_flight = in_flight;
        *this = e;
    }
};

constexpr uint32_t LINE_RING = 4;
template <class Rec>
struct DrawPassState {
    Rec* host[LINE_RING] = {}; size_t cap_host[LINE_RING] = {}; hipEvent_t ev[LINE_RING] = {}; uint32_t slot = 0;
    Rec* dev = nullptr; size_t cap_dev = 0;
    uint32_t *counters = nullptr, *lists = nullptr, *long_list = nullptr; size_t cap_tiles = 0; uint32_t parity = 0;
    unsigned long long tile_batches = 0, scan_batches = 0;
    void release() {
        for (uint32_t k = 0; k < LINE_RING; ++k) { if (ev[k]) (void)hipEventDestroy(ev[k]); if (host[k]) (void)hipHostFree(host[k]); }
        for (void* p : { (void*)dev, (void*)counters, (void*)lists, (void*)long_list }) if (p) (void)hipFree(p);
    }
};

struct TexSig { const void* ptr; uint32_t w, h, blend; uint64_t hash; };

struct b32_scene {
    B32Vertex* d_verts = nullptr; size_t cap_verts = 0;
    B32Face* d_faces = nullptr; size_t cap_faces = 0;
    uint16_t* d_texels = nullptr; size_t cap_texels = 0;
    uint32_t* d_texels32 = nullptr; size_t cap_texels32 = 0;
    TexDesc* d_tex = nullptr; size_t cap_tex = 0;
    std::vector<TexDesc> h_tex;
    uint32_t* d_consts = nullptr;
    uint8_t* d_atlas0 = nullptr; size_t cap_atlas0 = 0; uint32_t atlas_idx_bytes = 0;
    uint32_t* d_texmask = nullptr; size_t cap_texmask = 0;
    uint32_t pool_texels = 0; bool mask_dirty = true;
    uint32_t nv = 0, nf = 0, nt = 0;
    bool have_scene = false;
    unsigned long long gen = 0;
    bool fmt8 = false;
    bool blend8 = false;
    bool blend_texels8 = false;
    bool may_blend = true;
    bool cheap_ok = false;
    bool tex_blend_any = false;
    uint32_t blend_faces = 0;
    bool local_sort_ok = true;
    uint32_t direct_cap_opaque = 0;
    uint32_t direct_ntiles = 0;
    bool direct_ok = true;
    float* d_pos12 = nullptr; size_t cap_pos12 = 0; bool pos_valid = false; uint32_t band_frames = 0;
    bool lit_valid = false;
    std::vector<TexSig> tex_sig; bool tex_sig_valid = false;
    float* d_rest = nullptr; size_t cap_rest = 0; uint16_t* d_bone_of = nullptr; size_t cap_bone_of = 0; bool have_rig = false;
    void release() {
        for (void* p : { (void*)d_verts, (void*)d_faces, (void*)d_texels, (void*)d_texels32, (void*)d_tex, (void*)d_consts, (void*)d_texmask,
                         (void*)d_pos12, (void*)d_atlas0, (void*)d_rest, (void*)d_bone_of }) if (p) (void)hipFree(p);
    }
// ... 36 lines not shown
    uint32_t wire_seq = 0;
    bool start_lost = false;
    uint32_t join_seq = 0;
    uint32_t fill_seq = 0;
    bool pipe_hint = true;
    struct CoverOf { const Ctrl* ctrl; uint32_t tiles, groups, seq; } cover_of[3] = {};
    bool pipelined = false;
    unsigned long long pipelined_frames = 0;
    unsigned long long flag_join_frames = 0, event_join_frames = 0, poll_join_frames = 0;
    uint32_t inject = 0;

    uint32_t width = 0, height = 0;
    uint32_t* fb_own = nullptr; size_t fb_own_px = 0;
    uint32_t* fb = nullptr; bool fb_external = false;
    uint32_t band_y0 = 0, band_y1 = 0; bool band_set = false;
    float* zbuf = nullptr; size_t cap_zbuf = 0; bool zbuf_valid = false;

    void* band_fb_ipc = nullptr; uint32_t* band_sync_own = nullptr; uint32_t* band_sync = nullptr;
    uint32_t band_rank = 0; bool band_attached = false;

    b32_scene scene;
    int count_fragments = 0;
    bool last_exact = false;

    size_t cap_work = 0;
    uint32_t *keys1 = nullptr, *vals[2] = { nullptr, nullptr };
    uint32_t* counts = nullptr; uint32_t* block_sums = nullptr; uint32_t bin_blocks = 0;
    uint32_t* tile_mid = nullptr; size_t cap_tile_mid = 0;
    bool last_local_sort = false;
    uint32_t route_off = 0;
    uint32_t cheap_den = 64;
    size_t cap_pairs = 0;
    uint32_t* inline_lists = nullptr; size_t cap_inline = 0;
    bool last_direct = false;
    uint32_t epoch = 0;
    bool clear_pending = false; uint32_t clear_rgba = 0, clear_y0 = 0, clear_y1 = 0;
    unsigned long long routes[8] = {};
    unsigned long long lds_atlas_frames = 0;
    uint32_t *pkeys[2] = { nullptr, nullptr }, *pvals[2] = { nullptr, nullptr };
    uint32_t* block_hist = nullptr; uint32_t hist_blocks = 0; uint32_t* digit_total = nullptr;
    uint32_t partial_blocks = 0;
    uint32_t* ranges = nullptr; size_t cap_ranges = 0;
    uint32_t* vis = nullptr; size_t cap_vis = 0;
    uint32_t *wire_owner = nullptr, *wire_first = nullptr; size_t cap_wire_table = 0;
    unsigned long long wire_tile_frames = 0;
    DrawPassState<B32Line> lines;
    DrawPassState<B32Prim> prims;
    DrawPassState<B32WorldItem> world;
    ArmedWords world_counts;
    unsigned long long world_tile_batches = 0, world_scan_batches = 0;
    EventPair world_timer;
    DrawPassState<GizmoRow> gizmo; std::vector<GizmoRow> gizmo_rows;
    ArmedWords gizmo_counts;
    unsigned long long span_cover_frames = 0;
    Ctrl h_ctrl{}; Stamps h_stamps{};
    uint32_t h_consts[4] = { 0, 0, 0, 0 };
    bool defer_upload_sync = false;
    unsigned char* stage_host = nullptr; void* stage_dev = nullptr; size_t stage_cap = 0, stage_used = 0;
    bool stage_active = false, stage_failed = false; UploadSegs stage_segs{};
    B32Light* d_lights = nullptr; size_t cap_lights = 0; std::vector<B32Light> h_lights;

    bool frame_batched = false; MeshTable frame_table{};
    bool frame_placed = false; PlaceTable frame_places{};
    struct BatchEntry { b32_scene* slot; MeshRow row; bool wire; bool placed; B32Placement place; };
    struct MergedRun { std::vector<b32_scene*> members; std::vector<unsigned long long> gens; b32_scene* merged = nullptr; unsigned long long used = 0; };
    bool batch_open = false; B32Camera batch_cam{}; B32Settings batch_st{}; std::vector<B32Light> batch_lights; std::vector<BatchEntry> batch;
    std::vector<MergedRun> merged_runs; unsigned long long batch_clock = 0, gen_counter = 0;
    unsigned long long batch_stats[4] = {};
    bool frame_pending = false;
    bool pending_superseded = false;
    bool pending_may_redraw = false;
    bool deep_async = false;
    bool redrawing = false;
    int deferred_rc = 0;
    B32Camera last_cam{}; B32Settings last_settings{}; B32Fog last_fog{}; bool last_has_fog = false;

    static constexpr uint32_t DL_RING = 8;
    hipEvent_t dl_ev[DL_RING] = {}; unsigned long long dl_seq = 0;
    hipStream_t dl_stream = nullptr; hipEvent_t dl_snap[2] = {}; uint32_t* dl_stage[2] = {}; size_t dl_stage_px = 0;
    static constexpr uint32_t PICK_RING = 4;
    ArmedWords pick_words;
    DrawPassState<PickItem> pick_tab;
    void* pick_res[PICK_RING] = {}; size_t pick_cap_res[PICK_RING] = {}; hipEvent_t pick_done[PICK_RING] = {}, pick_left[PICK_RING] = {}; uint32_t pick_slot = 0;
    void* pick_host = nullptr; size_t pick_cap_host = 0;
    EventPair pick_timer;
    ArmedWords hover_bits, hover_words;
    EventPair hover_timer;
    ArmedWords room_words, room_points;
    uint4* overlay_tab = nullptr; size_t overlay_cap_tab = 0;
    void* overlay_bounds = nullptr;
    DrawPassState<uint32_t> overlay_sel; std::vector<uint32_t> overlay_pairs;
    int profile_level = 0;
    uint32_t prof_stride = 1, prof_seq = 0;
    hipEvent_t ev[EV_RING][EV_PER_FRAME] = {};
    bool ev_created = false;
    uint32_t ev_frames = 0;
    float phase_ms[5] = { 0, 0, 0, 0, 0 };
    uint32_t phase_frames = 0;
    int phase_level = 0;
    std::vector<B32Light> keep_lights;
};

#define HIPCHK(ctx, expr)                                                 \
    do {                                                                  \
        hipError_t _e = (expr);                                           \
        if (_e != hipSuccess) { (ctx)->last_hip = (int)_e; return B32_E_HIP; } \
// ... 97 lines not shown
```

bonnie-32_amd/csrc/b32_setup.hip:

```cpp
#include "b32_device.h"

namespace b32 {

struct UnrTable { uint8_t v[K::UNR_ENTRIES]; };
static constexpr UnrTable make_unr() {
    UnrTable t{};
    for (uint32_t i = 0; i < K::UNR_ENTRIES; ++i) {
        uint32_t q = K::UNR_NUMERATOR / (i + K::UNR_INDEX_OFFSET);
        int32_t val = (int32_t)((q + K::UNR_ROUND_ADD) / K::UNR_ROUND_DIV) - K::UNR_SUBTRACT;
        t.v[i] = val > 0 ? (uint8_t)val : 0;
    }
    return t;
}
__constant__ UnrTable g_unr = make_unr();

__device__ __forceinline__ int32_t wadd(int32_t a, int32_t b) { return (int32_t)((uint32_t)a + (uint32_t)b); }
__device__ __forceinline__ int32_t wsub(int32_t a, int32_t b) { return (int32_t)((uint32_t)a - (uint32_t)b); }
__device__ __forceinline__ int32_t fx_from_f32(float f) { return f2i32_sat(f * K::ONE_F); }
__device__ __forceinline__ int32_t fx_mul(int32_t a, int32_t b) { return (int32_t)(((int64_t)a * (int64_t)b) >> K::FRAC_BITS); }
struct UnrRecip { uint64_t nr2; uint32_t shift; bool neg, zero; };
__device__ __forceinline__ UnrRecip unr_recip(int32_t divisor, const uint8_t* __restrict__ table) {
    UnrRecip r;
    r.zero = divisor == 0; r.neg = divisor < 0;
    const uint32_t den = divisor < 0 ? (0u - (uint32_t)divisor) : (uint32_t)divisor;
// ... 125 lines not shown
    return rmin((z - start) / falloff, 1.0f);
}
__device__ __forceinline__ uint32_t fog_color(uint32_t c, uint32_t fogc, float f) {
    if (f <= 0.0f) return c;
    if (f >= 1.0f) return fogc;
    float inv = 1.0f - f;
    uint32_t o = 0;
#pragma unroll
    for (int i = 0; i < 3; ++i)
        o |= f2u8_sat((float)((c >> (8 * i)) & 255) * inv + (float)((fogc >> (8 * i)) & 255) * f) << (8 * i);
    return o;
}

struct AggSlot { uint32_t leader, rank, ret; };
__device__ __forceinline__ void agg_issue(uint32_t* fill, uint32_t slot, bool active, uint32_t lane, AggSlot& g) {
    g.leader = lane; g.rank = 0; g.ret = 0;
    uint32_t cnt = 1;
    unsigned long long rem = __ballot(active);
    const unsigned long long below = (1ull << lane) - 1ull;
    int misses = 0;
    for (int round = 0; round < 8 && rem; ++round) {
        const int l = __builtin_ctzll(rem);
        const uint32_t s = (uint32_t)__builtin_amdgcn_readlane((int)slot, l);
        const unsigned long long grp = __ballot(active && slot == s);
        rem &= ~grp;
        const uint32_t n = (uint32_t)__builtin_popcountll(grp);
        if (n < 2) { if (++misses >= 2) break; continue; }
        if (active && slot == s) { g.leader = (uint32_t)l; g.rank = (uint32_t)__builtin_popcountll(grp & below); if (lane == (uint32_t)l) cnt = n; }
    }
    if (active && g.leader == lane) g.ret = atomicAdd(fill + slot, cnt);
}
__device__ __forceinline__ uint32_t agg_position(const AggSlot& g) {
    return (uint32_t)__builtin_amdgcn_ds_bpermute((int)(g.leader << 2), (int)g.ret) + g.rank;
}

#ifndef B32_LIT_SETUP_WAVES
#define B32_LIT_SETUP_WAVES 6
#endif
struct FaceIn { uint32_t w[5]; float v[3][5]; uint32_t col[3]; bool live, bad; };
struct FaceMode { uint32_t tid, black_tr, face_blend, editor_alpha, tex_blend; bool have_tex; };
struct MeshParams { float ambient; bool cull, has_fog, placed; B32Fog fog; float cos, sin; V3 world; };
struct FaceAttr { float uvx[3], uvy[3]; uint32_t col[3]; V3 wn[3]; };
struct Winding { V3 v1, v2, v3; int i1, i2, i3; };
struct TriSetup {
    uint32_t min_x, max_x, min_y, max_y, bbx, bby;
    bool empty;
    float area, inv_area, a0, b0, a1, b1, w0_start, w1_start;
};
struct FaceOut {
    bool visible = false, transparent = false, nan_key = false, bad_index = false;
    uint32_t key = KEY_INVALID, span = 0xFFFFFFFFu, n_tiles = 0;
};

__device__ __forceinline__ void reset_frame(Ctrl* __restrict__ ctrl, const FrameParams& fp) {
    const bool lost = !fp.redraw && (ctrl->pairs_overflow || ctrl->need_global_sort);
    __syncthreads();
    if (threadIdx.x < sizeof(Ctrl) / 4 && threadIdx.x != offsetof(Ctrl, sticky) / 4) reinterpret_cast<uint32_t*>(ctrl)[threadIdx.x] = 0;
    if (threadIdx.x == 0 && lost) ctrl->sticky += 0x100u;
    if (threadIdx.x == 0) { Stamps* st = reinterpret_cast<Stamps*>(ctrl + 1); for (int k = 1; k < 8; ++k) st->t[k] = 0; st->t[ST_SETUP] = wall_clock64(); }
}

__device__ __forceinline__ FaceIn load_face(const SetupBuffers& a, const FrameParams& fp, uint32_t f) {
    FaceIn in;
    in.live = f < fp.nf; in.bad = false;
    if (in.live) {
        const uint32_t* fw = reinterpret_cast<const uint32_t*>(a.faces) + (size_t)f * 5;
#pragma unroll
        for (int k = 0; k < 5; ++k) in.w[k] = fw[k];
    }
    if (in.live) {
        in.bad = in.w[0] >= fp.nv || in.w[1] >= fp.nv || in.w[2] >= fp.nv;
        if (!in.bad) {
            if (a.pos12) {
#pragma unroll
                for (int j = 0; j < 3; ++j) {
                    const float* pp = a.pos12 + (size_t)in.w[j] * 3;
                    in.v[j][0] = pp[0]; in.v[j][1] = pp[1]; in.v[j][2] = pp[2];
                    in.v[j][3] = in.v[j][4] = 0.0f; in.col[j] = 0;
                }
            } else
#pragma unroll
            for (int j = 0; j < 3; ++j) {
                const float* vp = reinterpret_cast<const float*>(a.verts) + (size_t)in.w[j] * 9;
#pragma unroll
                for (int k = 0; k < 5; ++k) in.v[j][k] = vp[k];
                in.col[j] = reinterpret_cast<const uint32_t*>(vp)[8];
            }
        }
    }
    return in;
}

__device__ __forceinline__ MeshParams mesh_params(const FrameParams& fp, const MeshTable& mtab, const PlaceTable& ptab, uint32_t fb4) {
    MeshParams m = { fp.ambient, fp.backface_cull != 0, fp.has_fog != 0, false, fp.fog, 1.0f, 0.0f, { 0.0f, 0.0f, 0.0f } };
    if (fp.batched) {
        const MeshRow& mr = mtab.m[(fb4 >> 24) & (BATCH_MESHES - 1u)];
        m.ambient = mr.ambient; m.cull = (mr.flags & ROW_CULL) != 0; m.has_fog = (mr.flags & ROW_FOG) != 0; m.fog = mr.fog;
    }
    if (fp.placed) {
        const uint32_t mesh = fp.batched ? ((fb4 >> 24) & (BATCH_MESHES - 1u)) : 0u;
        m.placed = !fp.batched || (mtab.m[mesh].flags & ROW_PLACED) != 0;
        const B32Placement& pl = ptab.p[mesh];
        m.cos = pl.cos_f; m.sin = pl.sin_f; m.world = ld3(pl.world_pos);
    }
    return m;
}
// ... 104 lines not shown
                      __builtin_fabsf(p0 + q0) < L && __builtin_fabsf(p1 + q1) < L)) exact = false;
            }
    }
    return exact;
}

__device__ __forceinline__ void fetch_attributes(const SetupBuffers& a, const FrameParams& fp, const MeshParams& m, const uint32_t (&vi)[3],
                                                 const float (&camz)[3], FaceAttr& at) {
    if (a.pos12 && fp.shading != B32_SHADE_NONE) {
#pragma unroll
        for (int j = 0; j < 3; ++j) {
            const float* lp = a.attr12 + (size_t)fp.nv * 3 + (size_t)vi[j] * 6;
            at.uvx[j] = lp[0]; at.uvy[j] = lp[1]; at.col[j] = reinterpret_cast<const uint32_t*>(lp)[2];
            at.wn[j] = { lp[3], lp[4], lp[5] };
        }
    } else if (a.pos12) {
#pragma unroll
        for (int j = 0; j < 3; ++j) {
            const float* ap = a.attr12 + (size_t)vi[j] * 3;
            at.uvx[j] = ap[0]; at.uvy[j] = ap[1]; at.col[j] = reinterpret_cast<const uint32_t*>(ap)[2];
        }
    } else if (fp.shading != B32_SHADE_NONE) {
#pragma unroll
        for (int j = 0; j < 3; ++j) {
            const float* np = reinterpret_cast<const float*>(a.verts) + (size_t)vi[j] * 9 + 5;
            at.wn[j] = { np[0], np[1], np[2] };
        }
    }
    if (fp.placed && m.placed && fp.shading != B32_SHADE_NONE) {
#pragma unroll
        for (int j = 0; j < 3; ++j) at.wn[j] = { at.wn[j].x * m.cos - at.wn[j].z * m.sin, at.wn[j].y, at.wn[j].x * m.sin + at.wn[j].z * m.cos };
    }
    if (fp.has_fog && m.has_fog) {
        const uint32_t fogc = m.fog.r | (m.fog.g << 8) | (m.fog.b << 16) | ((uint32_t)m.fog.blend << 24);
#pragma unroll
        for (int j = 0; j < 3; ++j) at.col[j] = fog_color(at.col[j], fogc, fog_factor(camz[j], m.fog.start, m.fog.falloff));
    }
}

__device__ __forceinline__ uint32_t painter_key(float v1z, float v2z, float v3z, bool transparent, const FrameParams& fp, bool& nan_key) {
    float kz = (v1z + v2z + v3z) / 3.0f;
    if (fp.zmode && !transparent) kz = 0.0f;
    if (kz != kz) { nan_key = true; kz = 0.0f; }
    if (kz == 0.0f) kz = 0.0f;
    uint32_t zb = __float_as_uint(kz);
    uint32_t key = ((0x7FFFFFFFu - (zb & 0x7FFFFFFFu)) & 0x7FFFFFFFu) | (transparent ? 0x80000000u : 0u);
    if (fp.ortho) key = ~zsort_key(kz);
    if (fp.zmode && !transparent) key = 0;
    if (key == KEY_INVALID) key = 0xFFFFFFFEu;
    return key;
}

__device__ __forceinline__ void store_records(const RecArrays& recs, const FrameParams& fp, uint32_t rslot, const Winding& s, const TriSetup& t,
                                              const FaceMode& fm, const FaceAttr& at, uint32_t key, bool slow, bool transparent) {
    const V3 &v1 = s.v1, &v2 = s.v2, &v3 = s.v3;
    const int i1 = s.i1, i2 = s.i2, i3 = s.i3;
    const bool vc_diff = (at.col[i1] != at.col[i2]) || (at.col[i2] != at.col[i3]);
    const bool needs_dither = fp.dithering && (fp.shading == B32_SHADE_GOURAUD || fm.have_tex || vc_diff);
    const uint32_t eff_blend = fm.have_tex ? fm.tex_blend : fm.face_blend;
    const uint32_t flags = (fm.have_tex ? fm.tid : F_TEX_NONE) | (fm.black_tr ? F_BLACK_TR : 0) | (eff_blend << F_BLEND_SHIFT) |
                           (needs_dither ? F_DITHER : 0) | (slow ? F_SLOW : 0) | (transparent ? F_TRANSP : 0) |
                           (t.empty ? F_EMPTY : 0) | (fm.editor_alpha << F_ALPHA_SHIFT);
    const bool fits = !slow && max_abs_coord(s) <= 32767.0f;
    auto pk16 = [](float x, float y) { return ((uint32_t)(int32_t)x & 0xFFFFu) | ((uint32_t)(int32_t)y << 16); };
    uint4 c0, c1;
    c0.x = fits ? pk16(v1.x, v1.y) : COV_WIDE; c0.y = fits ? pk16(v2.x, v2.y) : 0u; c0.z = fits ? pk16(v3.x, v3.y) : 0u;
    c0.w = __float_as_uint(t.inv_area);
    c1 = make_uint4(t.bbx, t.bby, key, flags);
    uint4* cp = reinterpret_cast<uint4*>(recs.cov + rslot);
    cp[0] = c0; cp[1] = c1;
    const uint32_t slot = fm.have_tex ? fm.tid : F_TEX_NONE;
    const uint32_t shf = (fm.black_tr ? SH_BLACK_TR : 0u) | (needs_dither ? SH_DITHER : 0u) | (slow ? SH_SLOW : 0u);
    uint4* sp = reinterpret_cast<uint4*>(recs.shade + rslot);
    sp[0] = make_uint4(__float_as_uint(v1.x), __float_as_uint(v1.y), __float_as_uint(v2.x), __float_as_uint(v2.y));
    sp[1] = make_uint4(__float_as_uint(v3.x), __float_as_uint(v3.y), __float_as_uint(t.inv_area), (at.col[i1] & 0xFFFFFFu) | ((slot & 0xFFu) << 24));
    sp[2] = make_uint4(__float_as_uint(at.uvx[i1]), __float_as_uint(at.uvx[i2]), __float_as_uint(at.uvx[i3]), __float_as_uint(at.uvy[i1]));
    sp[3] = make_uint4(__float_as_uint(at.uvy[i2]), __float_as_uint(at.uvy[i3]), (at.col[i2] & 0xFFFFFFu) | ((slot >> 8) << 24), (at.col[i3] & 0xFFFFFFu) | (shf << 24));
    if (fp.zmode || !fp.affine || slow) {
        uint4* xp = reinterpret_cast<uint4*>(recs.aux + rslot);
        xp[0] = make_uint4(__float_as_uint(1.0f / v1.z), __float_as_uint(1.0f / v2.z), __float_as_uint(1.0f / v3.z), __float_as_uint(t.w0_start));
        xp[1] = make_uint4(__float_as_uint(t.w1_start), 0u, 0u, 0u);
    }
}

__device__ __forceinline__ void bin_span(const DirectBin& db, const FrameParams& fp, Ctrl* __restrict__ ctrl, uint32_t span, uint32_t n_tiles,
                                         bool db_cls, const AggSlot& first, uint32_t rslot) {
    const uint32_t cap = db_cls ? db.cap_transparent : db.cap_opaque;
    const uint32_t tx0 = span & 0xFF, tx1 = (span >> 8) & 0xFF, ty0 = (span >> 16) & 0xFF;
    bool over = false;
    uint32_t tx = tx0, ty = ty0;
    AggSlot g = first;
    for (uint32_t k = 0; __ballot(k < n_tiles); ++k) {
        const bool act = k < n_tiles;
        const uint32_t tile = ty * fp.tiles_x + tx;
        if (k) agg_issue(db.fill, tile * FILL_PAD + (db_cls ? 1u : 0u), act, threadIdx.x & 63u, g);
        const uint32_t pos = agg_position(g);
        if (act) {
            if (pos < cap) db.lists[(size_t)tile * db.region + (db_cls ? db.region - 1u - pos : pos)] = rslot;
            else over = true;
            if (++tx > tx1) { tx = tx0; ++ty; }
        }
    }
    if (over) { Events* ev = events_of(ctrl); if (db_cls) ev->long_transparent = db.epoch; else ev->overflow = db.epoch; }
}

__device__ __forceinline__ void store_shades(float* __restrict__ shades, const B32Light* lights, const FrameParams& fp, float ambient, uint32_t rslot,
                                             bool backface, const Winding& s, const V3 (&wpos)[3], V3 (&wn)[3]) {
    const int i1 = s.i1, i2 = s.i2, i3 = s.i3;
#pragma unroll
    for (int j = 0; j < 3; ++j) if (backface) wn[j] = scale3(wn[j], -1.0f);
    float* sh = shades + (size_t)rslot * 9;
    if (fp.shading == B32_SHADE_FLAT) {
        V3 center = scale3(add3(add3(wpos[i1], wpos[i2]), wpos[i3]), 1.0f / 3.0f);
        V3 nrm = normalize3(scale3(add3(add3(wn[i1], wn[i2]), wn[i3]), 1.0f / 3.0f));
        float c[3]; shade_multi(nrm, center, lights, fp.n_lights, ambient, c);
        for (int j = 0; j < 9; ++j) sh[j] = c[j % 3];
    } else {
        shade_multi(wn[i1], wpos[i1], lights, fp.n_lights, ambient, sh);
        shade_multi(wn[i2], wpos[i2], lights, fp.n_lights, ambient, sh + 3);
        shade_multi(wn[i3], wpos[i3], lights, fp.n_lights, ambient, sh + 6);
    }
}

__device__ __forceinline__ void publish_wave(const SetupBuffers& a, uint32_t f, bool live, const FaceOut& o, uint32_t (&wpart)[4][6]) {
    const unsigned long long mv = __ballot(o.visible), mt = __ballot(o.transparent);
    {
        const uint32_t lane = threadIdx.x & 63u, nvis = (uint32_t)__popcll(mv), wbase = f - lane;
        if (o.visible) {
            const uint32_t slot = wbase + (uint32_t)__popcll(mv & ((1ull << lane) - 1ull));
            a.keys[slot] = o.key;
            if (a.spans) a.spans[slot] = o.span;
            if (a.face_of) a.face_of[slot] = f;
        }
        if (live && lane >= nvis) { a.keys[wbase + lane] = KEY_INVALID; if (a.spans) a.spans[wbase + lane] = 0xFFFFFFFFu; }
    }
    const unsigned long long mn_op = __ballot(o.nan_key && !o.transparent), mn_tr = __ballot(o.nan_key && o.transparent), mb = __ballot(o.bad_index);
    const uint32_t wv = threadIdx.x >> 6;
    if ((threadIdx.x & 63) == 0) {
        wpart[wv][0] = (uint32_t)__popcll(mv); wpart[wv][1] = (uint32_t)__popcll(mt);
        wpart[wv][2] = (uint32_t)__popcll(mn_op); wpart[wv][3] = (uint32_t)__popcll(mn_tr); wpart[wv][4] = mb ? 1u : 0u;
        if (a.db.fill && (mn_op | mn_tr | mb)) {
            Events* ev = events_of(a.ctrl);
            if (mb) ev->bad_index = a.db.epoch;
            if (mn_op) ev->nan_opaque = a.db.epoch;
            if (mn_tr) ev->nan_transparent = a.db.epoch;
        }
    }
    uint32_t n_tiles = o.n_tiles;
    for (int off = 32; off > 0; off >>= 1) n_tiles += __shfl_down(n_tiles, off);
    if ((threadIdx.x & 63) == 0) wpart[wv][5] = n_tiles;
    __syncthreads();
    if (threadIdx.x < 6) a.partials[blockIdx.x * 8 + threadIdx.x] = wpart[0][threadIdx.x] + wpart[1][threadIdx.x] + wpart[2][threadIdx.x] + wpart[3][threadIdx.x];
// ... 2 lines not shown
template <int PLAIN>
__global__ __launch_bounds__(256) __attribute__((amdgpu_waves_per_eu(PLAIN == 1 ? 8 : (PLAIN == 2 ? B32_LIT_SETUP_WAVES : 4), PLAIN == 1 ? 8 : (PLAIN == 2 ? B32_LIT_SETUP_WAVES : 5)))) void k_setup(SetupArgs args) {
    FrameParams fp = args.fp;
    if (PLAIN) { fp.ortho = 0; fp.fixed_point = 1; fp.has_fog = 0; fp.wire_collect = 0; fp.xray = 0; fp.batched = 0; fp.placed = 0; }
    if (PLAIN == 1) { fp.shading = B32_SHADE_NONE; fp.n_lights = 0; }
    __shared__ uint32_t wpart[4][6];
    __shared__ uint8_t unr_lds[K::UNR_ENTRIES + 3];
    for (uint32_t i = threadIdx.x; i < K::UNR_ENTRIES; i += 256) unr_lds[i] = g_unr.v[i];
    __syncthreads();
    const SetupBuffers b = args.buf;
    const B32Light* lights = fp.lights_inline ? args.lset.l : b.lights;
    if (blockIdx.x == 0) reset_frame(b.ctrl, fp);
    const uint32_t f = blockIdx.x * 256u + threadIdx.x;
    const FaceIn in = load_face(b, fp, f);
    FaceOut out;
    if (in.live) {
        const uint32_t vi[3] = { in.w[0], in.w[1], in.w[2] }, fb4 = in.w[4];
        FaceMode fm = { in.w[3], fb4 & 0xFF, (fb4 >> 8) & 0xFF, (fb4 >> 16) & 0xFF, B32_BLEND_OPAQUE, false };
        const MeshParams mp = mesh_params(fp, args.mtab, args.ptab, fb4);
        if (in.bad) {
            out.bad_index = true;
        } else {
            V3 scr[3], wpos[3]; float camz[3];
            FaceAttr at = {};
#pragma unroll
            for (int j = 0; j < 3; ++j) {
                wpos[j] = place_vertex(fp, mp, { in.v[j][0], in.v[j][1], in.v[j][2] });
                at.uvx[j] = in.v[j][3]; at.uvy[j] = in.v[j][4]; at.col[j] = in.col[j];
                scr[j] = project_vertex(fp, wpos[j], unr_lds, camz[j]);
            }
            bool backface;
            if (cull_face(b, fp, mp, f, scr, camz, fm, backface)) {
                out.visible = true;
                const uint32_t rslot = (f & ~63u) + (uint32_t)__builtin_popcountll(__ballot(true) & ((1ull << (threadIdx.x & 63u)) - 1ull));
                out.transparent = (fm.have_tex && fm.tex_blend != B32_BLEND_OPAQUE) || fm.face_blend != B32_BLEND_OPAQUE || fm.editor_alpha < 255;
                if (fp.fmt8) out.transparent = false;
                const int i2 = backface ? 2 : 1, i3 = backface ? 1 : 2;
                const Winding s = { scr[0], scr[i2], scr[i3], 0, i2, i3 };
                TriSetup t = triangle_prologue(fp, s, out.span, out.n_tiles);
                AggSlot db_first = { 0, 0, 0 }; bool db_cls = false;
                if (b.db.fill && out.n_tiles) {
                    db_cls = b.db.with_class && out.transparent;
                    const uint32_t t0 = ((out.span >> 16) & 0xFF) * fp.tiles_x + (out.span & 0xFF);
                    agg_issue(b.db.fill, t0 * FILL_PAD + (db_cls ? 1u : 0u), true, threadIdx.x & 63u, db_first);
                }
                const bool need_rec = !fp.band_only || out.n_tiles != 0;
                bool slow = !fp.fixed_point || fp.ortho;
                if (need_rec) {
                    fetch_attributes(b, fp, mp, vi, camz, at);
                    triangle_edges(s, t);
                    if (!slow && !t.empty) slow = !walk_is_exact(s, t);
                }
                out.key = painter_key(s.v1.z, s.v2.z, s.v3.z, out.transparent, fp, out.nan_key);
                if (need_rec) store_records(b.recs, fp, rslot, s, t, fm, at, out.key, slow, out.transparent);
                if (b.db.fill && out.n_tiles) bin_span(b.db, fp, b.ctrl, out.span, out.n_tiles, db_cls, db_first, rslot);
                if (need_rec && fp.shading != B32_SHADE_NONE) store_shades(b.shades, lights, fp, mp.ambient, rslot, backface, s, wpos, at.wn);
            }
        }
        if (fp.wire_collect && out.bad_index) b.wire[f].kind = 0;
    }
    publish_wave(b, f, in.live, out, wpart);
}

void launch_setup(hipStream_t s, const SetupArgs& a) {
    const FrameParams& fp = a.fp;
    if (fp.nf == 0) return;
    const bool plain = fp.fixed_point && !fp.ortho && !fp.has_fog && !fp.wire_collect && fp.shading == B32_SHADE_NONE && !fp.xray && !fp.batched && !fp.placed;
    const dim3 g1((fp.nf + 255) / 256);
    const bool lit = fp.fixed_point && !fp.ortho && !fp.has_fog && !fp.wire_collect && fp.shading != B32_SHADE_NONE && !fp.xray && !fp.batched && !fp.placed;
    if (lit) hipLaunchKernelGGL(k_setup<2>, g1, dim3(256), 0, s, a);
    else if (plain) hipLaunchKernelGGL(k_setup<1>, g1, dim3(256), 0, s, a);
    else hipLaunchKernelGGL(k_setup<0>, g1, dim3(256), 0, s, a);
}

__global__ void k_merge_mesh(const B32Vertex* __restrict__ sv, uint32_t nv, const B32Face* __restrict__ sf, uint32_t nf, uint32_t nt,
                             B32Vertex* __restrict__ dv, B32Face* __restrict__ df, uint32_t vbase, uint32_t tbase, uint32_t mesh) {
    const uint32_t i = blockIdx.x * blockDim.x + threadIdx.x;
    if (i < nv) {
        const uint32_t* s = reinterpret_cast<const uint32_t*>(sv) + (size_t)i * 9;
        uint32_t* d = reinterpret_cast<uint32_t*>(dv) + (size_t)(vbase + i) * 9;
#pragma unroll
        for (int k = 0; k < 9; ++k) d[k] = s[k];
    }
    if (i < nf) {
        const uint32_t* s = reinterpret_cast<const uint32_t*>(sf) + (size_t)i * 5;
        uint32_t* d = reinterpret_cast<uint32_t*>(df) + (size_t)i * 5;
#pragma unroll
        for (int k = 0; k < 3; ++k) d[k] = s[k] < nv ? s[k] + vbase : 0xFFFFFFFFu;
        d[3] = (s[3] != B32_NO_TEXTURE && s[3] < nt) ? s[3] + tbase : B32_NO_TEXTURE;
        d[4] = (s[4] & 0x00FFFFFFu) | (mesh << 24);
    }
}
void launch_merge_mesh(hipStream_t s, const B32Vertex* sv, uint32_t nv, const B32Face* sf, uint32_t nf, uint32_t nt, B32Vertex* dv, B32Face* df,
                       uint32_t vbase, uint32_t tbase, uint32_t mesh) {
    const uint32_t n = nv > nf ? nv : nf;
    if (n) hipLaunchKernelGGL(k_merge_mesh, dim3((n + 255) / 256), dim3(256), 0, s, sv, nv, sf, nf, nt, dv, df, vbase, tbase, mesh);
}
__global__ void k_offset_tex(const TexDesc* __restrict__ src, uint32_t nt, TexDesc* __restrict__ dst, uint32_t texel_base) {
    const uint32_t i = blockIdx.x * blockDim.x + threadIdx.x;
    if (i < nt) { TexDesc d = src[i]; d.offset += texel_base; dst[i] = d; }
}
void launch_offset_tex(hipStream_t s, const TexDesc* src, uint32_t nt, TexDesc* dst, uint32_t texel_base) {
    if (nt) hipLaunchKernelGGL(k_offset_tex, dim3((nt + 255) / 256), dim3(256), 0, s, src, nt, dst, texel_base);
}

__global__ void k_gate(Ctrl* __restrict__ prev, uint32_t need, uint32_t patience, uint32_t start_seq, Ctrl* __restrict__ mine, uint32_t start_patience) {
    if (start_seq) {
        const unsigned long long t0 = wall_clock64();
// ... 193 lines not shown
```

bonnie-32_amd/csrc/b32_shade_tile.h:

```cpp
#pragma once
#include "b32_fill_common.h"

namespace b32 {

template <bool FMT8, bool ZMODE>
__device__ __forceinline__ void repair_pixel(const FillArgs& a, const unsigned long long* sec, bool need, uint32_t row, uint32_t col, uint32_t px, uint32_t py,
                                             uint32_t e0, uint32_t e1, uint32_t lane, bool& ok, Hit& h, unsigned long long& t) {
    const uint32_t W = a.fp.width;
    auto sid_of = [](unsigned long long v) { return ZMODE ? 0xFFFFFFFEu - (uint32_t)v : (uint32_t)v; };
    unsigned long long limit = 0, seed = 0;
    if (need) {
        if (ZMODE) seed = ((unsigned long long)(~zsort_key(a.clear_depth ? __uint_as_float(0x7F7FFFFFu) : a.zbuf[(size_t)py * W + px])) << 32) | 0xFFFFFFFFull;
        const unsigned long long t2 = sec[row * STR64 + col];
        if (t2 > seed) {
            ok = hit_test<FMT8>(a, sid_of(t2), px, py, h);
            if (ok) t = t2; else limit = t2;
        }
    }
    unsigned long long fm = __ballot(limit != 0);
    while (fm) {
        const int fl = __builtin_ctzll(fm);
        fm &= fm - 1;
        const uint32_t fx = (uint32_t)__builtin_amdgcn_readlane((int)px, fl), fy = (uint32_t)__builtin_amdgcn_readlane((int)py, fl);
        const unsigned long long lim = ((unsigned long long)(uint32_t)__builtin_amdgcn_readlane((int)(limit >> 32), fl) << 32) |
                                       (uint32_t)__builtin_amdgcn_readlane((int)(uint32_t)limit, fl);
        const unsigned long long sd = ((unsigned long long)(uint32_t)__builtin_amdgcn_readlane((int)(seed >> 32), fl) << 32) |
                                      (uint32_t)__builtin_amdgcn_readlane((int)(uint32_t)seed, fl);
        unsigned long long best = 0;
        for (uint32_t base = e0; base < e1; base += 64) {
            unsigned long long cand = 0;
            if (base + lane < e1) {
                const uint32_t csid = a.pair_vals[base + lane];
                const uint4 cc1 = reinterpret_cast<const uint4*>(a.crecs + csid)[1];
                const uint32_t bbx = cc1.x, bby = cc1.y;
                if (fx >= (bbx & 0xFFFF) && fx < (bbx >> 16) && fy >= (bby & 0xFFFF) && fy < (bby >> 16)) {
                    unsigned long long P = ((unsigned long long)cc1.z << 32) | csid;
                    Hit c;
                    if (ZMODE) {
                        if (hit_test<FMT8>(a, csid, fx, fy, c) && depth_prio(a, csid, c, P) && P < lim && P > sd) cand = P;
                    } else if (P < lim && P > best && hit_test<FMT8>(a, csid, fx, fy, c)) cand = P;
                }
            }
            for (int off = 32; off > 0; off >>= 1) { const unsigned long long o = __shfl_xor(cand, off); cand = o > cand ? o : cand; }
            best = cand > best ? cand : best;
        }
        if ((int)lane == fl && best) { ok = hit_test<FMT8>(a, sid_of(best), px, py, h); t = best; }
    }
}

template <bool FMT8, int NT, bool ZMODE>
__device__ __forceinline__ void shade_tile_p64(const FillArgs& a, const uint32_t* tilebuf, uint32_t e0, uint32_t e1, const TileRect& rect,
                                               uint32_t tid_in, uint32_t lane_in, uint32_t* wq, const uint8_t* latlas) {
    const uint32_t x_lo = rect.x_lo, x_hi = rect.x_hi, y_lo = rect.y_lo, y_hi = rect.y_hi, ty_top = rect.ty_top, TH = rect.th;
    uint32_t tid = tid_in, lane = lane_in;
    asm volatile("" : "+v"(tid), "+v"(lane));
    const FrameParams& fp = a.fp;
    const unsigned long long* top = reinterpret_cast<const unsigned long long*>(tilebuf);
    const unsigned long long* sec = top + TILE_H * STR64;
    const int shading = fp.shading;
    const bool need5 = !fp.affine || !fp.fixed_point || fp.ortho;
    const uint32_t W = fp.width;
    constexpr uint32_t ROWS_PER_STEP = NT / 64;
    auto covered = [](unsigned long long t) { return ZMODE ? ((uint32_t)t != 0xFFFFFFFFu) : (t != 0ull); };
    auto sid_of = [](unsigned long long t) { return ZMODE ? 0xFFFFFFFEu - (uint32_t)t : (uint32_t)t; };
    auto put = [&](uint32_t px, uint32_t py, bool ok, const Hit& h, unsigned long long t, bool in) {
        if (ok) {
            a.fb[(size_t)py * W + px] = colour<FMT8>(a, h, shading, px, py);
            if (ZMODE) { float z = zsort_val(~(uint32_t)(t >> 32)); if (z == 0.0f) z = exact_depth_at(a, h.sid, px, py); a.zbuf[(size_t)py * W + px] = z; }
        } else if (in) {
            if (a.clear_on) a.fb[(size_t)py * W + px] = a.clear_rgba;
            if (ZMODE && a.clear_depth) a.zbuf[(size_t)py * W + px] = __uint_as_float(0x7F7FFFFFu);
        }
    };
    uint32_t lqn = 0;
    auto drain = [&]() {
        const bool act = lane < lqn;
        const uint32_t e = act ? wq[lane] : 0u;
        const uint32_t row = e >> 6, col = e & 63u, px = x_lo + col, py = ty_top + row;
        bool ok = false; Hit h; h.sid = 0;
        unsigned long long t = 0;
        repair_pixel<FMT8, ZMODE>(a, sec, act, row, col, px, py, e0, e1, lane, ok, h, t);
        if (act) put(px, py, ok, h, t, true);
        lqn = 0;
    };
    const unsigned long long below = (1ull << lane) - 1ull;
    for (uint32_t r0 = 0; r0 < TH; r0 += 2 * ROWS_PER_STEP) {
// ... 218 lines not shown
```

bonnie-32_amd/rasterizer.py:

```python
import ctypes as C

import numpy as np

from . import abi
from . import rtypes as T


class B32Error(RuntimeError):
    def __init__(self, code, where=""):
        self.code = code
        msg = abi.load_library().b32_strerror(code).decode()
        super().__init__(f"{where}: {msg} (code {code})" if where else f"{msg} (code {code})")


def _chk(rc, where=""):
    if rc != abi.B32_OK:
        raise B32Error(rc, where)


def place_vertices(vertices, cos_f, sin_f, world_pos):
    v = np.array(vertices, dtype=abi.VERTEX_DTYPE, copy=True)
    c, s = np.float32(cos_f), np.float32(sin_f)
    w = np.asarray(world_pos, np.float32).reshape(3)
    with np.errstate(all="ignore"):
# ... 942 lines not shown
        return self.buf[:48].view(abi.ROOM_HOVER_DTYPE)[0].copy()

    close = HoverResult.close


def _pack_placement(placement):
    if placement is None or isinstance(placement, abi.B32Placement):
        return placement
    return placement.pack()


class Context:

    def __init__(self, device=0):
        self.lib = abi.load_library()
        h = C.c_void_p()
        _chk(self.lib.b32_create(device, C.byref(h)), "b32_create")
        self.h = h
        self.device = device

    def close(self):
        if getattr(self, "h", None):
            self.lib.b32_destroy(self.h)
            self.h = None

    def __del__(self):
        try:
            self.close()
        except Exception:
            pass

    def set_stream(self, stream_ptr):
        HIP_STREAM_LEGACY = 1
        _chk(self.lib.b32_set_stream(self.h, stream_ptr if stream_ptr else HIP_STREAM_LEGACY), "b32_set_stream")

    def use_own_stream(self):
        _chk(self.lib.b32_set_stream(self.h, None), "b32_set_stream")

    def synchronize(self):
        _chk(self.lib.b32_synchronize(self.h), "b32_synchronize")

    def set_profiling(self, level):
        _chk(self.lib.b32_set_profiling(self.h, level), "b32_set_profiling")

    def set_profiling_stride(self, every):
        _chk(self.lib.b32_set_profiling_stride(self.h, int(every)), "b32_set_profiling_stride")

    def set_async_depth(self, deep):
        _chk(self.lib.b32_set_async_depth(self.h, int(deep)), "b32_set_async_depth")

    ROUTES = ("direct_bin", "inline_bin", "counting_sort", "keyed", "redraw_region", "redraw_global_sort", "redraw_pairs", "pipelined", "lds_atlas", "wire_tiles", "span_cover",
              "flag_join", "event_join", "poll_join", "line_tiles", "line_scan", "prim_tiles", "prim_scan")
    WORLD_ROUTES = ("world_tiles", "world_scan")

    ROUTE_SORT_FREE, ROUTE_CUT_TILES, ROUTE_INLINE_BIN, ROUTE_DIRECT_BIN, ROUTE_WIDE_GROUPS, ROUTE_PACKED_STREAMS, ROUTE_PIPELINE, ROUTE_TEX_CACHE, ROUTE_BATCH, ROUTE_LDS_ATLAS, ROUTE_WIRE_TILES, ROUTE_SPAN_COVER, ROUTE_STAGGER, ROUTE_LINE_TILES, ROUTE_PRIM_TILES = 1, 2, 4, 8, 16, 32, 64, 128, 256, 512, 1024, 2048, 4096, 8192, 16384

    def frame_begin(self, camera, settings):
        cam = camera.pack()
        st, keep = settings.pack()
        self._frame_keep = (cam, st, keep)
        _chk(self.lib.b32_frame_begin(self.h, C.byref(cam), C.byref(st)), "b32_frame_begin")

    def frame_add(self, scene, ambient=None, backface_cull=None, backface_wireframe=None, fog=None, placement=None):
        st = self._frame_keep[1]
        p = abi.B32MeshParams()
        p.ambient = float(st.ambient if ambient is None else ambient)
        p.backface_cull = int(st.backface_cull if backface_cull is None else bool(backface_cull))
        p.backface_wireframe = int(st.backface_wireframe if backface_wireframe is None else bool(backface_wireframe))
        fg = T.pack_fog(fog)
        p.has_fog = 0 if fg is None else 1
        if fg is not None:
            p.fog = fg
        scene.detach()
        if placement is not None:
            pl = _pack_placement(placement)
            _chk(self.lib.b32_frame_add_scene_placed(self.h, scene._slot, C.byref(p), C.byref(pl) if pl is not None else None), "b32_frame_add_scene_placed")
            return
        _chk(self.lib.b32_frame_add_scene(self.h, scene._slot, C.byref(p)), "b32_frame_add_scene")

    def frame_end(self):
        _chk(self.lib.b32_frame_end(self.h), "b32_frame_end")

    def frame_submit(self, table):
        if len(table) == 8:
            cam, st, _keep, slots, params, n, places, has_place = table
            _chk(self.lib.b32_frame_submit_placed(self.h, C.byref(cam), C.byref(st), slots, C.cast(params, C.c_void_p), C.cast(places, C.c_void_p),
                                                  C.cast(has_place, C.c_void_p), n), "b32_frame_submit_placed")
            return
        cam, st, _keep, slots, params, n = table
        _chk(self.lib.b32_frame_submit(self.h, C.byref(cam), C.byref(st), slots, C.cast(params, C.c_void_p), n), "b32_frame_submit")

    @staticmethod
    def set_table_placements(table, placements):
        places, has_place = table[6], table[7]
        for i, pl in enumerate(placements):
            p = _pack_placement(pl)
            has_place[i] = 0 if p is None else 1
            if p is not None:
                places[i] = p

    @staticmethod
    def make_frame_table(camera, settings, scenes, fogs=None, ambients=None, placements=None, backface_culls=None):
        cam = camera.pack()
        st, keep = settings.pack()
        n = len(scenes)
        slots = (C.c_void_p * n)()
# ... 219 lines not shown
        return int(t.value), BoxResult(arr, (self, ptr) if own else None)

    def finish(self) -> T.RasterTimings:
        tm = abi.B32Timings()
        _chk(self.lib.b32_frame_finish(self.h, C.byref(tm)), "b32_frame_finish")
        return T.RasterTimings.from_c(tm)

    def batch_counts(self):
        return {n: int(self.lib.b32_batch_count(self.h, i)) for i, n in enumerate(("merged_draws", "single_draws", "merged_built", "frames"))}

    def set_pipeline_gate(self, permille):
        _chk(self.lib.b32_set_pipeline_gate(self.h, int(permille)), "b32_set_pipeline_gate")

    def last_shader_clock(self):
        g, m = C.c_float(), C.c_float()
        _chk(self.lib.b32_last_shader_clock(self.h, C.byref(g), C.byref(m)), "b32_last_shader_clock")
        return float(g.value), float(m.value)

    def transparent_counts(self):
        a, b = C.c_uint32(), C.c_uint32()
        _chk(self.lib.b32_transparent_counts(self.h, C.byref(a), C.byref(b)), "b32_transparent_counts")
        return int(a.value), int(b.value)

    def set_pipeline_depth(self, sets):
        _chk(self.lib.b32_set_pipeline_depth(self.h, int(sets)), "b32_set_pipeline_depth")

    def mesh_overlay_record_count(self, topology, nv, overlay, selected=None):
        o, sel = overlay.pack(selected)
        n = C.c_uint32()
        _chk(self.lib.b32_mesh_overlay_record_count(topology.handle(self) if topology is not None else None, nv, C.byref(o),
                                                    abi.ptr(sel) if len(sel) else None, C.byref(n)), "mesh_overlay_record_count")
        return int(n.value)

    def gizmo_project_batch(self, items, camera: T.Camera, ortho, width, height):
        arr = np.ascontiguousarray(items, dtype=abi.GIZMO_ITEM_DTYPE).reshape(-1)
        cap = int(sum(gizmo_record_count(int(k), min(int(s), abi.GIZMO_MAX_THICKNESS)) for k, s in zip(arr["kind"], arr["size"])))
        out = np.zeros(cap, abi.PRIM_DTYPE)
        cam = camera.pack()
        o = _pack_ortho(ortho)
        n = C.c_uint32()
        _chk(self.lib.b32_gizmo_project_batch(self.h, C.byref(cam), C.byref(o) if o is not None else None, arr.ctypes.data if len(arr) else None,
                                              len(arr), int(width), int(height), out.ctypes.data if cap else None, cap, C.byref(n)),
             "gizmo_project_batch")
        return out[:int(n.value)]

    def set_routes(self, off_mask):
        _chk(self.lib.b32_set_routes(self.h, int(off_mask)), "b32_set_routes")

    def set_cheap_threshold(self, den):
        _chk(self.lib.b32_set_cheap_threshold(self.h, int(den)), "b32_set_cheap_threshold")

    def route_counts(self):
        return {n: int(self.lib.b32_route_count(self.h, i)) for i, n in enumerate(self.ROUTES + self.WORLD_ROUTES)}

    def debug_inject(self, what):
        _chk(self.lib.b32_debug_inject(self.h, int(what)), "b32_debug_inject")

    def set_fragment_counting(self, on):
        _chk(self.lib.b32_set_fragment_counting(self.h, int(on)), "b32_set_fragment_counting")

    def last_kernel_times(self):
        names = (C.c_char_p * 8)()
        ms = (C.c_float * 8)()
        n = self.lib.b32_last_kernel_times(self.h, names, ms, 8)
        return {names[i].decode(): float(ms[i]) for i in range(n)}

    BAND_SHARE_BYTES = 96

    def band_export(self) -> bytes:
        buf = C.create_string_buffer(self.BAND_SHARE_BYTES)
        _chk(self.lib.b32_band_export(self.h, C.cast(buf, C.c_void_p)), "b32_band_export")
        return buf.raw

    def band_import(self, share: bytes, rank):
        assert len(share) == self.BAND_SHARE_BYTES
        buf = C.create_string_buffer(share, self.BAND_SHARE_BYTES)
        rc = self.lib.b32_band_import(self.h, C.cast(buf, C.c_void_p), int(rank))
        _chk(rc, f"b32_band_import (hip error {self.lib.b32_last_hip_error(self.h)})" if rc else "b32_band_import")
        w, h = np.frombuffer(share, np.uint32, 2, 64)
        return int(w), int(h)

    def band_attach(self, root: "Context", rank):
        _chk(self.lib.b32_band_attach(self.h, root.h, int(rank)), "b32_band_attach")

    def band_close(self):
        _chk(self.lib.b32_band_close(self.h), "b32_band_close")

    def band_publish(self, frame_no):
        _chk(self.lib.b32_band_publish(self.h, int(frame_no)), "b32_band_publish")

    def band_wait(self, rank, frame_no, timeout_us=2_000_000):
        _chk(self.lib.b32_band_wait(self.h, int(rank), int(frame_no), int(timeout_us)), "b32_band_wait")

    def band_wait_all(self, nranks, frame_no, timeout_us=2_000_000, release_after=True):
        _chk(self.lib.b32_band_wait_all(self.h, int(nranks), int(frame_no), int(timeout_us), 1 if release_after else 0), "b32_band_wait_all")

    def band_release(self, frame_no):
        _chk(self.lib.b32_band_release(self.h, int(frame_no)), "b32_band_release")

    def band_acquire(self, frame_no, timeout_us=2_000_000):
        _chk(self.lib.b32_band_acquire(self.h, int(frame_no), int(timeout_us)), "b32_band_acquire")

    def band_status(self):
        ep = (C.c_uint32 * 64)(); root = C.c_uint32(); to = C.c_uint32()
        _chk(self.lib.b32_band_status(self.h, ep, C.byref(root), C.byref(to)), "b32_band_status")
        return list(ep), int(root.value), int(to.value)
# ... 972 lines not shown
```

include/b32raster.h:

```cpp
#ifndef B32RASTER_H
#define B32RASTER_H

#include <stddef.h>
#include <stdint.h>

#ifdef __cplusplus
extern "C" {
#endif

#define B32_OK             0
#define B32_E_ARG         -1
#define B32_E_INDEX       -2
#define B32_E_NAN_KEY     -3
#define B32_E_HIP         -4
#define B32_E_UNSUPPORTED -5
#define B32_E_NO_DEVICE   -6
#define B32_E_FRAME_DROPPED -7
#define B32_E_BAND_TIMEOUT -8

#define B32_BLEND_OPAQUE      0
#define B32_BLEND_AVERAGE     1
#define B32_BLEND_ADD         2
#define B32_BLEND_SUBTRACT    3
#define B32_BLEND_ADD_QUARTER 4
// ... 110 lines not shown
int b32_fb_upload(b32_ctx* ctx, const uint8_t* rgba);
int b32_fb_download(b32_ctx* ctx, uint8_t* rgba);
void* b32_host_alloc(size_t bytes);
void b32_host_free(void* p);
int b32_fb_download_async(b32_ctx* ctx, uint8_t* rgba, uint64_t* ticket);
int b32_ticket_poll(b32_ctx* ctx, uint64_t ticket, int* done);
int b32_ticket_wait(b32_ctx* ctx, uint64_t ticket);
int b32_zbuffer_download(b32_ctx* ctx, float* z);
int b32_zbuffer_upload(b32_ctx* ctx, const float* z);
int b32_fb_bind_device(b32_ctx* ctx, void* device_rgba, uint32_t width, uint32_t height);
int b32_fb_size(const b32_ctx* ctx, uint32_t* width, uint32_t* height);
int b32_set_band(b32_ctx* ctx, uint32_t y0, uint32_t y1);

int b32_render_mesh_15(b32_ctx* ctx,
                       const B32Vertex* vertices, uint32_t nv,
                       const B32Face* faces, uint32_t nf,
                       const B32Texture15* textures, uint32_t nt,
                       const B32Camera* camera, const B32Settings* settings,
                       const B32Fog* fog ,
                       B32Timings* out );

int b32_scene_upload(b32_ctx* ctx,
                     const B32Vertex* vertices, uint32_t nv,
                     const B32Face* faces, uint32_t nf,
                     const B32Texture15* textures, uint32_t nt);
int b32_scene_upload_indexed(b32_ctx* ctx,
                             const B32Vertex* vertices, uint32_t nv,
                             const B32Face* faces, uint32_t nf,
                             const B32IndexedTexture* textures, uint32_t nt);
int b32_render_scene_15(b32_ctx* ctx,
                        const B32Camera* camera, const B32Settings* settings,
                        const B32Fog* fog ,
                        B32Timings* out );
int b32_render_scene_15_async(b32_ctx* ctx,
                              const B32Camera* camera, const B32Settings* settings,
                              const B32Fog* fog );
int b32_frame_finish(b32_ctx* ctx, B32Timings* out );
int b32_set_async_depth(b32_ctx* ctx, int deep);
unsigned long long b32_route_count(const b32_ctx* ctx, int which);
#define B32_ROUTE_SORT_FREE   1u
#define B32_ROUTE_CUT_TILES   2u
#define B32_ROUTE_INLINE_BIN  4u
#define B32_ROUTE_DIRECT_BIN  8u
#define B32_ROUTE_WIDE_GROUPS 16u
#define B32_ROUTE_PACKED_STREAMS 32u
#define B32_ROUTE_TEX_CACHE   128u
#define B32_ROUTE_BATCH       256u
#define B32_ROUTE_LDS_ATLAS   512u
#define B32_ROUTE_WIRE_TILES  1024u
#define B32_ROUTE_SPAN_COVER  2048u
#define B32_ROUTE_STAGGER     4096u
#define B32_ROUTE_LINE_TILES  8192u
#define B32_ROUTE_PRIM_TILES 16384u
#define B32_ROUTE_PIPELINE    64u
int b32_set_routes(b32_ctx* ctx, uint32_t off_mask);
int b32_set_cheap_threshold(b32_ctx* ctx, uint32_t den);

typedef struct b32_scene b32_scene;
int b32_scene_create(b32_ctx* ctx, b32_scene** out);
void b32_scene_destroy(b32_ctx* ctx, b32_scene* slot);
int b32_scene_swap(b32_ctx* ctx, b32_scene* slot);

typedef struct B32Bone {
    float pos[3];
    float cos_x, sin_x, cos_z, sin_z;
    uint32_t rotate;
} B32Bone;
#define B32_BONE_NONE 0xFFFFu
#define B32_MAX_BONES 64u
int b32_scene_set_rig(b32_ctx* ctx, b32_scene* slot , const uint16_t* bone_of_vertex );
int b32_scene_pose(b32_ctx* ctx, b32_scene* slot , const B32Bone* bones, uint32_t n_bones);
int b32_scene_read_vertices(b32_ctx* ctx, b32_scene* slot , uint32_t first, uint32_t count, B32Vertex* out);

typedef struct B32MeshParams {
    float   ambient;
    uint8_t backface_cull, backface_wireframe, has_fog, _pad;
    B32Fog  fog;
} B32MeshParams;
int b32_frame_begin(b32_ctx* ctx, const B32Camera* camera, const B32Settings* base_settings);
int b32_frame_add_scene(b32_ctx* ctx, b32_scene* slot, const B32MeshParams* params );
int b32_frame_end(b32_ctx* ctx);
int b32_frame_submit(b32_ctx* ctx, const B32Camera* camera, const B32Settings* base_settings, b32_scene* const* slots,
                     const B32MeshParams* params , uint32_t n);
unsigned long long b32_batch_count(const b32_ctx* ctx, int which);

typedef struct B32Placement {
    float cos_f, sin_f;
    float world_pos[3];
} B32Placement;
int b32_frame_add_scene_placed(b32_ctx* ctx, b32_scene* slot, const B32MeshParams* params , const B32Placement* place );
int b32_frame_submit_placed(b32_ctx* ctx, const B32Camera* camera, const B32Settings* base_settings, b32_scene* const* slots,
                            const B32MeshParams* params , const B32Placement* places ,
                            const uint8_t* has_place , uint32_t n);
int b32_render_scene_15_placed_async(b32_ctx* ctx, const B32Camera* camera, const B32Settings* settings, const B32Fog* fog ,
                                     const B32Placement* place );

typedef struct B32PickHit { uint32_t hit; uint32_t tri; float depth; uint32_t _pad; } B32PickHit;
#define B32_PICK_CULL_BACKFACES 1u
struct B32Ortho;
int b32_pick_meshes(b32_ctx* ctx, const B32Camera* camera, const struct B32Ortho* ortho , float mx, float my, uint32_t flags,
                    b32_scene* const* slots, const B32Placement* places , uint32_t n,
                    B32PickHit* hits , int32_t* best );
int b32_pick_meshes_async(b32_ctx* ctx, const B32Camera* camera, const struct B32Ortho* ortho , float mx, float my, uint32_t flags,
                          b32_scene* const* slots, const B32Placement* places , uint32_t n,
                          void* out , uint64_t* ticket);

// ... 264 lines not shown
```

Measured before the change: 9843 Mtriangles/s.

## Store coverage records inline in per-tile opaque lists instead of indices

When direct binning is active, the setup kernel writes a 32-byte coverage record (vertex coords, bbox, key, flags, slot id) straight into each tile's opaque list. The global coverage-record write is skipped for opaque fast triangles. The fill and shade-tile passes then read these records sequentially instead of chasing an index into the crecs array, and narrow triangles recompute the inverse area from the edge terms. This removes a dependent scattered load per list entry, at the cost of duplicating records for every tile a triangle touches, which means more write bandwidth and up to 1 GiB of extra buffer.

```diff
diff --git a/bonnie-32_amd/csrc/b32_api.hip b/bonnie-32_amd/csrc/b32_api.hip
--- a/bonnie-32_amd/csrc/b32_api.hip
+++ b/bonnie-32_amd/csrc/b32_api.hip
@@ -882,6 +882,7 @@
     if (c && which == 17) return c->prims.scan_batches;
     if (c && which == 18) return c->world_tile_batches;
     if (c && which == 19) return c->world_scan_batches;
+    if (c && which == 20) return c->record_list_frames;
     return (c && which >= 0 && which < 8) ? c->routes[which] : 0ull;
 }
 extern "C" int b32_set_async_depth(b32_ctx* c, int deep) {
diff --git a/bonnie-32_amd/csrc/b32_cover.h b/bonnie-32_amd/csrc/b32_cover.h
--- a/bonnie-32_amd/csrc/b32_cover.h
+++ b/bonnie-32_amd/csrc/b32_cover.h
@@ -229,7 +229,7 @@
         Batch b;
         uint32_t my_sid = 0, my_key = 0;
         bool narrow = false;
-        load_batch<TEXMODE>(b, a, e0 + e, live, lds_desc, EXACT, ZMODE || (EXACT && !affine), my_sid, my_key, narrow);
+        load_batch<TEXMODE, P64>(b, a, e0 + e, live, lds_desc, EXACT, ZMODE || (EXACT && !affine), my_sid, my_key, narrow);
         if (ZMODE) { my_key = 0u; my_sid = 0xFFFFFFFEu - my_sid; }
         const uint32_t flags = b.q3.w;
         const uint32_t cx0 = max(b.q1.w & 0xFFFF, x_lo), cx1 = min(b.q1.w >> 16, x_hi);
diff --git a/bonnie-32_amd/csrc/b32_device.h b/bonnie-32_amd/csrc/b32_device.h
--- a/bonnie-32_amd/csrc/b32_device.h
+++ b/bonnie-32_amd/csrc/b32_device.h
@@ -100,6 +100,11 @@
     view_edges(r, i16lo(c0.x), i16hi(c0.x), i16lo(c0.y), i16hi(c0.y), i16lo(c0.z), i16hi(c0.z), __uint_as_float(c0.w));
     return true;
 }
+__device__ __forceinline__ float rcp_exact(float x);
+__device__ __forceinline__ float list_rec_inv_area(const RecView& r) {
+    const float a0 = __uint_as_float(r.q0.z), b0 = __uint_as_float(r.q0.w), a1 = __uint_as_float(r.q1.x), b1 = __uint_as_float(r.q1.y);
+    return rcp_exact(a0 * b1 + b0 * -a1);
+}
 __device__ __forceinline__ void view_edges_from_shade(RecView& r, const uint4& s0, const uint4& s1) {
     view_edges(r, __uint_as_float(s0.x), __uint_as_float(s0.y), __uint_as_float(s0.z), __uint_as_float(s0.w), __uint_as_float(s1.x),
                __uint_as_float(s1.y), __uint_as_float(s1.z));
@@ -316,6 +321,7 @@
 struct DirectBin {
     uint32_t* fill;
     uint32_t* lists;
+    uint4* rec;
     uint32_t region, cap_opaque, cap_transparent;
     uint32_t with_class;
     uint32_t epoch;
@@ -485,6 +491,8 @@
     uint32_t inline_bin;
     uint32_t direct_bin;
     uint32_t* tile_fill;
+    const uint4* rec_lists;
+    uint32_t opaque_stride;
     uint32_t epoch;
     uint32_t list_stride;
     const uint32_t* spans;
diff --git a/bonnie-32_amd/csrc/b32_fill.hip b/bonnie-32_amd/csrc/b32_fill.hip
--- a/bonnie-32_amd/csrc/b32_fill.hip
+++ b/bonnie-32_amd/csrc/b32_fill.hip
@@ -113,9 +113,9 @@
     } else if (P64 && a.direct_bin) {
         const uint32_t* fl = a.tile_fill + (size_t)tile * FILL_PAD;
         const uint32_t n_o = fl[0], n_t = fl[1];
-        e0 = tile * a.list_stride; e1 = e0 + n_o;
+        e0 = tile * a.opaque_stride; e1 = e0 + n_o;
         if (tid == 0) {
-            if (a.gather_blend) a.tile_mid[tile] = e0 + a.list_stride - n_t;
+            if (a.gather_blend) a.tile_mid[tile] = (tile + 1u) * a.list_stride - n_t;
             if (n_o | n_t) atomicAdd(&a.ctrl->n_pairs, n_o + n_t);
         }
     } else if (P64) {
diff --git a/bonnie-32_amd/csrc/b32_fill_common.h b/bonnie-32_amd/csrc/b32_fill_common.h
--- a/bonnie-32_amd/csrc/b32_fill_common.h
+++ b/bonnie-32_amd/csrc/b32_fill_common.h
@@ -263,26 +263,26 @@
     }
     if (sh & SH_SLOW) { const uint4 c1 = reinterpret_cast<const uint4*>(a.crecs + sid)[1]; r.q1.w = c1.x; r.q2.x = c1.y; }
 }
-__device__ __forceinline__ void load_full_view(const FillArgs& a, uint32_t sid, RecView& r) {
-    load_shade_view(a, sid, true, r);
-    const uint4 c1 = reinterpret_cast<const uint4*>(a.crecs + sid)[1];
-    r.q1.w = c1.x; r.q2.x = c1.y; r.q3.w = c1.w;
-}
-
-template <int TEXMODE>
+
+template <int TEXMODE, bool P64>
 __device__ __forceinline__ void load_batch(Batch& b, const FillArgs& a, uint32_t entry, bool live, const TexDesc& lds_desc, bool need_uv,
                                            bool need_aux, uint32_t& sid_out, uint32_t& key_out, bool& narrow_out) {
     b.q0 = b.q1 = b.q2 = b.q3 = b.q4 = b.q5 = make_uint4(0, 0, 0, 0);
     b.tw = b.th = b.toff = 0;
     sid_out = 0; key_out = 0; narrow_out = false;
     if (live) {
-        const uint32_t sid = a.pair_vals[entry];
-        const uint4* cp = reinterpret_cast<const uint4*>(a.crecs + sid);
+        const bool rec = P64 && a.rec_lists != nullptr;
+        uint32_t sid = 0;
+        const uint4* cp;
+        if (rec) cp = a.rec_lists + 2 * (size_t)entry;
+        else { sid = a.pair_vals[entry]; cp = reinterpret_cast<const uint4*>(a.crecs + sid); }
         const uint4 c0 = cp[0], c1 = cp[1];
+        if (rec) sid = c0.w;
         sid_out = sid; key_out = c1.z;
         RecView v;
         v.q0 = v.q1 = v.q2 = v.q3 = v.q4 = v.q5 = make_uint4(0, 0, 0, 0);
         const bool narrow = view_from_cov(v, c0, c1);
+        if (rec && narrow) v.q1.z = __float_as_uint(list_rec_inv_area(v));
         narrow_out = narrow;
         if (!narrow || need_uv) {
             const uint4* sp = reinterpret_cast<const uint4*>(a.srecs + sid);
@@ -361,7 +361,7 @@
 
 __device__ inline float exact_depth_at(const FillArgs& a, uint32_t sid, uint32_t px, uint32_t py) {
     RecView rv;
-    load_full_view(a, sid, rv);
+    load_shade_view(a, sid, true, rv);
     const Tri tr = tri_from_view(rv, true);
     float w0, w1, bcx, bcy, bcz;
     edge_w(tr, px, py, w0, w1);
diff --git a/bonnie-32_amd/csrc/b32_frame.hip b/bonnie-32_amd/csrc/b32_frame.hip
--- a/bonnie-32_amd/csrc/b32_frame.hip
+++ b/bonnie-32_amd/csrc/b32_frame.hip
@@ -66,6 +66,7 @@
     bool local_sort = false;
     bool want_inline = false;
     bool direct_bin = false;
+    bool record_lists = false;
     bool inline_bin = false, prio64 = false;
     uint32_t list_stride = 0;
     DirectBin db{};
@@ -246,8 +247,17 @@
                 HIPCHK(c, hipMemsetAsync(c->cur.tile_fill, 0, c->cur.cap_tile_fill * sizeof(uint32_t), c->stream));
                 c->side_dirty = true;
             }
+            r.record_lists = plan_record_lists(true, ntiles, cap_o, (c->route_off & B32_ROUTE_RECORD_LISTS) != 0);
+            if (r.record_lists) {
+                const size_t need_rec = (size_t)ntiles * cap_o + 2;
+                if (need_rec > c->cur.cap_rec || !c->cur.rec_lists) {
+                    if ((rc = ensure_plain(c, c->cur.rec_lists, 2 * (need_rec + need_rec / 8)))) return rc;
+                    c->cur.cap_rec = need_rec + need_rec / 8;
+                }
+            }
             if (++c->epoch == 0) c->epoch = 1;
             r.db.fill = c->cur.tile_fill; r.db.lists = c->cur.direct_lists; r.db.region = region; r.db.cap_opaque = cap_o;
+            r.db.rec = r.record_lists ? c->cur.rec_lists : nullptr;
             r.db.cap_transparent = r.with_class ? BLEND_SORT_CAP : 0u; r.db.with_class = r.with_class ? 1u : 0u; r.db.epoch = c->epoch;
             r.direct_bin = true;
             r.list_stride = region;
@@ -348,6 +358,7 @@
     if (r.inline_bin) fa.pair_vals = c->inline_lists;
     fa.direct_bin = r.direct_bin ? 1u : 0u; fa.tile_fill = c->cur.tile_fill; fa.epoch = c->epoch;
     if (r.direct_bin) fa.pair_vals = c->cur.direct_lists;
+    fa.rec_lists = r.record_lists ? c->cur.rec_lists : nullptr; fa.opaque_stride = r.record_lists ? r.db.cap_opaque : r.list_stride;
     fa.gather_blend = (r.prio64 && r.with_class) ? 1u : 0u;
     fa.stagger = (c->route_off & B32_ROUTE_STAGGER) ? 0u : 1u;
     fa.span_cover = (r.prio64 && !r.exact_cov && !fp.zmode && !(c->route_off & B32_ROUTE_SPAN_COVER)) ? 1u : 0u;
@@ -501,6 +512,7 @@
                                       c->tile_mid, BLEND_SORT_CAP, c->pvals[0]));
     if (!r.prio64 && (rc = bin_keyed(c, fp, r, sc, r.prof_all ? r.ev[2] : nullptr))) return rc;
     c->routes[r.direct_bin ? 0 : r.inline_bin ? 1 : r.prio64 ? 2 : 3]++;
+    if (r.record_lists) c->record_list_frames++;
     const bool direct_safe = r.direct_bin && r.db.cap_opaque >= c->scene.nf && (!r.with_class || c->scene.blend_faces <= BLEND_SORT_CAP);
     c->pending_may_redraw = !(r.inline_bin || direct_safe);
     if (r.prof_fill) HIPCHK(c, hipEventRecord(r.ev[3], s));
diff --git a/bonnie-32_amd/csrc/b32_frame_plan.h b/bonnie-32_amd/csrc/b32_frame_plan.h
--- a/bonnie-32_amd/csrc/b32_frame_plan.h
+++ b/bonnie-32_amd/csrc/b32_frame_plan.h
@@ -28,6 +28,13 @@
 
 inline bool plan_wide(uint32_t ntiles, uint32_t n_cu, bool narrow_only) { return ntiles <= n_cu && !narrow_only; }
 
+constexpr uint64_t RECORD_LIST_ENTRY_BYTES = 32;
+constexpr uint64_t RECORD_LIST_MAX_BYTES = (uint64_t)1 << 30;
+inline uint64_t plan_record_list_bytes(uint32_t ntiles, uint32_t cap_opaque) { return (uint64_t)ntiles * cap_opaque * RECORD_LIST_ENTRY_BYTES; }
+inline bool plan_record_lists(bool direct_bin, uint32_t ntiles, uint32_t cap_opaque, bool route_off) {
+    return direct_bin && !route_off && ntiles != 0 && cap_opaque != 0 && plan_record_list_bytes(ntiles, cap_opaque) <= RECORD_LIST_MAX_BYTES;
+}
+
 inline bool plan_pipe_hint(bool direct_bin, uint32_t ntiles, uint32_t n_cu, bool batched, bool join_small) {
     return direct_bin && (ntiles > 2u * n_cu || batched || join_small);
 }
diff --git a/bonnie-32_amd/csrc/b32_host.h b/bonnie-32_amd/csrc/b32_host.h
--- a/bonnie-32_amd/csrc/b32_host.h
+++ b/bonnie-32_amd/csrc/b32_host.h
@@ -23,6 +23,7 @@
     uint32_t* face_of = nullptr;
     float* shades = nullptr; size_t cap_shades = 0;
     uint32_t* direct_lists = nullptr; size_t cap_direct = 0;
+    uint4* rec_lists = nullptr; size_t cap_rec = 0;
     uint32_t* tile_fill = nullptr; size_t cap_tile_fill = 0;
     WireTri* wire = nullptr; size_t cap_wire = 0;
     uint32_t *wire_fill = nullptr, *wire_lists = nullptr; size_t cap_wire_tiles = 0;
@@ -32,7 +33,7 @@
     bool in_flight = false;
     void release() {
         for (void* p : { (void*)keys0, (void*)crecs, (void*)srecs, (void*)xrecs, (void*)spans, (void*)face_of, (void*)partials, (void*)shades,
-                         (void*)direct_lists, (void*)tile_fill, (void*)wire, (void*)wire_fill, (void*)wire_lists }) if (p) (void)hipFree(p);
+                         (void*)direct_lists, (void*)rec_lists, (void*)tile_fill, (void*)wire, (void*)wire_fill, (void*)wire_lists }) if (p) (void)hipFree(p);
         FrameSet e; e.d_ctrl = d_ctrl; e.ev_setup = ev_setup; e.in_flight = in_flight;
         *this = e;
     }
@@ -175,6 +176,7 @@
     EventPair world_timer;
     DrawPassState<GizmoRow> gizmo; std::vector<GizmoRow> gizmo_rows;
     ArmedWords gizmo_counts;
+    unsigned long long record_list_frames = 0;
     unsigned long long span_cover_frames = 0;
     Ctrl h_ctrl{}; Stamps h_stamps{};
     uint32_t h_consts[4] = { 0, 0, 0, 0 };
diff --git a/bonnie-32_amd/csrc/b32_setup.hip b/bonnie-32_amd/csrc/b32_setup.hip
--- a/bonnie-32_amd/csrc/b32_setup.hip
+++ b/bonnie-32_amd/csrc/b32_setup.hip
@@ -201,6 +201,8 @@
     uint32_t key = KEY_INVALID, span = 0xFFFFFFFFu, n_tiles = 0;
 };
 
+struct ListEntry { uint32_t xy1 = 0, xy2 = 0, xy3 = 0, bbx = 0, bby = 0, flags = 0; };
+
 __device__ __forceinline__ void reset_frame(Ctrl* __restrict__ ctrl, const FrameParams& fp) {
     const bool lost = !fp.redraw && (ctrl->pairs_overflow || ctrl->need_global_sort);
     __syncthreads();
@@ -411,7 +413,8 @@
 }
 
 __device__ __forceinline__ void store_records(const RecArrays& recs, const FrameParams& fp, uint32_t rslot, const Winding& s, const TriSetup& t,
-                                              const FaceMode& fm, const FaceAttr& at, uint32_t key, bool slow, bool transparent) {
+                                              const FaceMode& fm, const FaceAttr& at, uint32_t key, bool slow, bool transparent, bool rec_lists,
+                                              ListEntry& le) {
     const V3 &v1 = s.v1, &v2 = s.v2, &v3 = s.v3;
     const int i1 = s.i1, i2 = s.i2, i3 = s.i3;
     const bool vc_diff = (at.col[i1] != at.col[i2]) || (at.col[i2] != at.col[i3]);
@@ -426,8 +429,11 @@
     c0.x = fits ? pk16(v1.x, v1.y) : COV_WIDE; c0.y = fits ? pk16(v2.x, v2.y) : 0u; c0.z = fits ? pk16(v3.x, v3.y) : 0u;
     c0.w = __float_as_uint(t.inv_area);
     c1 = make_uint4(t.bbx, t.bby, key, flags);
-    uint4* cp = reinterpret_cast<uint4*>(recs.cov + rslot);
-    cp[0] = c0; cp[1] = c1;
+    le.xy1 = c0.x; le.xy2 = c0.y; le.xy3 = c0.z; le.bbx = c1.x; le.bby = c1.y; le.flags = c1.w;
+    if (!(rec_lists && !transparent && !slow)) {
+        uint4* cp = reinterpret_cast<uint4*>(recs.cov + rslot);
+        cp[0] = c0; cp[1] = c1;
+    }
     const uint32_t slot = fm.have_tex ? fm.tid : F_TEX_NONE;
     const uint32_t shf = (fm.black_tr ? SH_BLACK_TR : 0u) | (needs_dither ? SH_DITHER : 0u) | (slow ? SH_SLOW : 0u);
     uint4* sp = reinterpret_cast<uint4*>(recs.shade + rslot);
@@ -443,7 +449,7 @@
 }
 
 __device__ __forceinline__ void bin_span(const DirectBin& db, const FrameParams& fp, Ctrl* __restrict__ ctrl, uint32_t span, uint32_t n_tiles,
-                                         bool db_cls, const AggSlot& first, uint32_t rslot) {
+                                         bool db_cls, const AggSlot& first, uint32_t rslot, uint32_t key, const ListEntry& le) {
     const uint32_t cap = db_cls ? db.cap_transparent : db.cap_opaque;
     const uint32_t tx0 = span & 0xFF, tx1 = (span >> 8) & 0xFF, ty0 = (span >> 16) & 0xFF;
     bool over = false;
@@ -455,8 +461,11 @@
         if (k) agg_issue(db.fill, tile * FILL_PAD + (db_cls ? 1u : 0u), act, threadIdx.x & 63u, g);
         const uint32_t pos = agg_position(g);
         if (act) {
-            if (pos < cap) db.lists[(size_t)tile * db.region + (db_cls ? db.region - 1u - pos : pos)] = rslot;
-            else over = true;
+            if (pos >= cap) over = true;
+            else if (db.rec && !db_cls) {
+                uint4* ep = db.rec + 2 * ((size_t)tile * db.cap_opaque + pos);
+                ep[0] = make_uint4(le.xy1, le.xy2, le.xy3, rslot); ep[1] = make_uint4(le.bbx, le.bby, key, le.flags);
+            } else db.lists[(size_t)tile * db.region + (db_cls ? db.region - 1u - pos : pos)] = rslot;
             if (++tx > tx1) { tx = tx0; ++ty; }
         }
     }
@@ -565,8 +574,9 @@
                     if (!slow && !t.empty) slow = !walk_is_exact(s, t);
                 }
                 out.key = painter_key(s.v1.z, s.v2.z, s.v3.z, out.transparent, fp, out.nan_key);
-                if (need_rec) store_records(b.recs, fp, rslot, s, t, fm, at, out.key, slow, out.transparent);
-                if (b.db.fill && out.n_tiles) bin_span(b.db, fp, b.ctrl, out.span, out.n_tiles, db_cls, db_first, rslot);
+                ListEntry le;
+                if (need_rec) store_records(b.recs, fp, rslot, s, t, fm, at, out.key, slow, out.transparent, b.db.rec != nullptr, le);
+                if (b.db.fill && out.n_tiles) bin_span(b.db, fp, b.ctrl, out.span, out.n_tiles, db_cls, db_first, rslot, out.key, le);
                 if (need_rec && fp.shading != B32_SHADE_NONE) store_shades(b.shades, lights, fp, mp.ambient, rslot, backface, s, wpos, at.wn);
             }
         }
diff --git a/bonnie-32_amd/csrc/b32_shade_tile.h b/bonnie-32_amd/csrc/b32_shade_tile.h
--- a/bonnie-32_amd/csrc/b32_shade_tile.h
+++ b/bonnie-32_amd/csrc/b32_shade_tile.h
@@ -30,8 +30,11 @@
         for (uint32_t base = e0; base < e1; base += 64) {
             unsigned long long cand = 0;
             if (base + lane < e1) {
-                const uint32_t csid = a.pair_vals[base + lane];
-                const uint4 cc1 = reinterpret_cast<const uint4*>(a.crecs + csid)[1];
+                uint32_t csid;
+                const uint4* cq;
+                if (a.rec_lists) { cq = a.rec_lists + 2 * (size_t)(base + lane); csid = cq[0].w; }
+                else { csid = a.pair_vals[base + lane]; cq = reinterpret_cast<const uint4*>(a.crecs + csid); }
+                const uint4 cc1 = cq[1];
                 const uint32_t bbx = cc1.x, bby = cc1.y;
                 if (fx >= (bbx & 0xFFFF) && fx < (bbx >> 16) && fy >= (bby & 0xFFFF) && fy < (bby >> 16)) {
                     unsigned long long P = ((unsigned long long)cc1.z << 32) | csid;
diff --git a/bonnie-32_amd/rasterizer.py b/bonnie-32_amd/rasterizer.py
--- a/bonnie-32_amd/rasterizer.py
+++ b/bonnie-32_amd/rasterizer.py
@@ -1018,6 +1018,7 @@
     ROUTES = ("direct_bin", "inline_bin", "counting_sort", "keyed", "redraw_region", "redraw_global_sort", "redraw_pairs", "pipelined", "lds_atlas", "wire_tiles", "span_cover",
               "flag_join", "event_join", "poll_join", "line_tiles", "line_scan", "prim_tiles", "prim_scan")
     WORLD_ROUTES = ("world_tiles", "world_scan")
+    ROUTE_RECORD_LISTS = 32768
 
     ROUTE_SORT_FREE, ROUTE_CUT_TILES, ROUTE_INLINE_BIN, ROUTE_DIRECT_BIN, ROUTE_WIDE_GROUPS, ROUTE_PACKED_STREAMS, ROUTE_PIPELINE, ROUTE_TEX_CACHE, ROUTE_BATCH, ROUTE_LDS_ATLAS, ROUTE_WIRE_TILES, ROUTE_SPAN_COVER, ROUTE_STAGGER, ROUTE_LINE_TILES, ROUTE_PRIM_TILES = 1, 2, 4, 8, 16, 32, 64, 128, 256, 512, 1024, 2048, 4096, 8192, 16384
 
@@ -1343,6 +1344,9 @@
 
     def route_counts(self):
         return {n: int(self.lib.b32_route_count(self.h, i)) for i, n in enumerate(self.ROUTES + self.WORLD_ROUTES)}
+
+    def record_list_frames(self):
+        return int(self.lib.b32_route_count(self.h, 20))
 
     def debug_inject(self, what):
         _chk(self.lib.b32_debug_inject(self.h, int(what)), "b32_debug_inject")
diff --git a/include/b32raster.h b/include/b32raster.h
--- a/include/b32raster.h
+++ b/include/b32raster.h
@@ -186,6 +186,7 @@
 #define B32_ROUTE_STAGGER     4096u
 #define B32_ROUTE_LINE_TILES  8192u
 #define B32_ROUTE_PRIM_TILES 16384u
+#define B32_ROUTE_RECORD_LISTS 32768u
 #define B32_ROUTE_PIPELINE    64u
 int b32_set_routes(b32_ctx* ctx, uint32_t off_mask);
 int b32_set_cheap_threshold(b32_ctx* ctx, uint32_t den);
```

Result: no change. 9904 Mtriangles/s, median of 2 (+0.6%).
